# ModelTC/llmc

Hardware: AMD Instinct MI355X
Metric: layers/sec (GPTQ W4A16, Llama-3-8B Linear shapes, 128x2048 calib) (higher is better)
Workload: dtype bf16

## Files before the change

### llmc_amd/_ffi.py

```python
import ctypes as C
import os

import torch

_HERE = os.path.dirname(os.path.abspath(__file__))
LIB_PATH = os.path.join(_HERE, 'csrc', 'libllmc_hip.so')

F16, BF16, F32 = 0, 1, 2
F64 = 3
OUT_FAKE, OUT_I32, OUT_I8, OUT_U8 = 0, 1, 2, 3
SCALAR_QPARAM = 16
LINEAR_YBLOCKED = 4
FRACTIONAL_ZP = 32
KV_REQUANT, KV_NEW_FAKE = 1, 2

_DT = {torch.float16: F16, torch.bfloat16: BF16, torch.float32: F32}

_i64, _i32, _f32, _f64, _vp, _sz = C.c_int64, C.c_int, C.c_float, C.c_double, C.c_void_p, C.c_size_t

SIGNATURES = {
    'llmc_hip_abi_version': (_i32, []),
    'llmc_hip_build_id': (C.c_char_p, []),
    'llmc_hip_last_error': (_i32, [C.c_char_p, _sz]),
    'llmc_hip_set_helper_streams': (_i32, [_i32]),
    'llmc_hip_set_cu_reserve': (_i32, [_i32]),
    'llmc_hip_set_option': (_i32, [C.c_char_p, _i32]),
    'llmc_hip_get_option': (_i32, [C.c_char_p]),
    'llmc_hip_option_name': (_i32, [_i32, C.c_char_p, _sz]),
    'llmc_minmax_qparams_ws_bytes': (_sz, [_i64, _i64]),
    'llmc_minmax_qparams': (_i32, [_vp, _i32, _i64, _i64, _i32, _i32, _f32, _f32, _vp, _vp, _vp, _vp]),
    'llmc_minmax_samples_max': (_i32, []),
    'llmc_minmax_samples_ws_bytes': (_sz, [_vp, _i32]),
    'llmc_minmax_samples': (_i32, [_vp, _vp, _i32, _i32, _vp, _vp, _vp, _vp]),
    'llmc_histc_ws_bytes': (_sz, [_i32]),
    'llmc_histc': (_i32, [_vp, _i32, _i64, _i32, _f32, _f32, _vp, _vp, _vp]),
    'llmc_mse_qparams': (_i32, [_vp, _i32, _i64, _i64, _i32, _i32, _f32, _f32, _i32, _i32, _f32, _vp, _vp, _vp, _vp, _vp]),
    'llmc_mse_qparams_panel': (_i32, [_vp, _i64, _i64, _i64, _i64, _i64, _i32, _i32, _f32, _f32, _i32, _i32, _f32, _vp,
                                      _vp, _i64, _i64, _vp]),
    'llmc_hqq_ws_bytes': (_sz, [_i64, _i64, _i32, _i64, _i32]),
    'llmc_hqq_optimize': (_i32, [_vp, _i32, _i64, _i64, _i64, _i32, _i64, _i32, _i32, _f32, _f32, _vp, _vp, _f32, _f32,
                                 _i32, _i32, _vp, _vp, _vp, _vp, _vp, _vp]),
    'llmc_quant_static': (_i32, [_vp, _i32, _i64, _i64, _vp, _i32, _vp, _i32, _f32, _f32, _i32, _vp, _vp]),
    'llmc_quant_dynamic_ws_bytes': (_sz, [_i64, _i64]),
    'llmc_quant_dynamic': (_i32, [_vp, _i32, _i64, _i64, _i32, _i32, _f32, _f32, _i32, _vp, _vp, _vp, _vp, _vp]),
    'llmc_pack_lsb': (_i32, [_vp, _i32, _i64, _i64, _i32, _vp, _vp]),
    'llmc_hessian_accum_ws_bytes': (_sz, [_i64, _i64, _i64]),
    'llmc_hessian_accum': (_i32, [_vp, _vp, _i32, _i64, _i64, _i64, _f64, _f64, _vp, _vp]),
    'llmc_hessian_accum_partials': (_i32, [_vp, _i32, _i64, _i64, _i64, _vp, _vp]),
    'llmc_hessian_accum_reduce': (_i32, [_vp, _i64, _i64, _i64, _f64, _f64, _vp, _vp]),
    'llmc_hessian_max_samples': (_i32, []),
    'llmc_hessian_accum_ptrs_ws_bytes': (_sz, [_vp, _i32, _i64, _i64]),
    'llmc_hessian_accum_ptrs': (_i32, [_vp, _vp, _vp, _i32, _i32, _i64, _i64, _f64, _f64, _vp, _vp]),
    'llmc_hessian_accum_ptrs_partials': (_i32, [_vp, _vp, _i32, _i32, _i64, _i64, _vp, _vp]),
    'llmc_hessian_accum_ptrs_reduce': (_i32, [_vp, _vp, _i32, _i64, _i64, _f64, _f64, _vp, _vp]),
    'llmc_hessian_accum_barrier_timeouts': (_i32, [_vp, _vp, _i32, _i64, _i64, _vp, _vp]),
    'llmc_hessian_max_problems': (_i32, []),
    'llmc_hessian_accum_multi_ws_bytes': (_sz, [_vp, _i32]),
    'llmc_hessian_accum_multi_partials': (_i32, [_vp, _i32, _i32, _vp, _vp]),
    'llmc_hessian_accum_multi_reduce': (_i32, [_vp, _i32, _vp, _vp]),
    'llmc_hessian_accum_multi_barrier_timeouts': (_i32, [_vp, _i32, _vp, _vp, _vp]),
    'llmc_gather_cols': (_i32, [_vp, _i64, _i64, _vp, _vp, _vp]),
    'llmc_hessian_prep_ws_bytes': (_sz, [_i64]),
    'llmc_hessian_prep': (_i32, [_vp, _vp, _i32, _i64, _i64, _vp, _f32, _vp, _vp, _vp, _vp]),
    'llmc_chol_inv_upper_ws_bytes': (_sz, [_i64]),
    'llmc_chol_inv_upper': (_i32, [_vp, _i64, _vp, _vp, _vp]),
    'llmc_hessian_prep_rev': (_i32, [_vp, _vp, _i32, _i64, _i64, _vp, _f32, _vp, _vp, _vp, _vp]),
    'llmc_chol_inv_upper_rev': (_i32, [_vp, _vp, _i64, _vp, _vp, _vp]),
    'llmc_gptq_quantize_ws_bytes': (_sz, [_i64, _i64]),
    'llmc_gptq_quantize': (_i32, [_vp, _vp, _i64, _i64, _i32, _f32, _f32, _i64, _i32, _vp, _vp, _vp, _vp, _vp,
                                  _i32, _vp, _vp]),
    'llmc_gptq_quantize_cols': (_i32, [_vp, _vp, _i64, _i64, _i64, _i32, _f32, _f32, _i64, _i32, _vp, _vp, _vp, _vp, _vp,
                                       _i32, _vp, _vp]),
    'llmc_gptq_quantize_fp8_cols': (_i32, [_vp, _vp, _i64, _i64, _i64, _i32, _i64, _i32, _vp, _vp, _vp, _vp, _i32, _vp, _vp]),
    'llmc_gptq_quantize_mse_ws_bytes': (_sz, [_i64, _i64]),
    'llmc_gptq_quantize_mse': (_i32, [_vp, _vp, _i64, _i64, _i64, _i32, _f32, _f32, _i64, _i32, _i32, _i32, _f32, _vp, _vp,
                                      _vp, _vp, _i32, _vp, _vp]),
    'llmc_spqr_quantize_ws_bytes': (_sz, [_i64, _i64]),
    'llmc_spqr_quantize': (_i32, [_vp, _vp, _i64, _i64, _f32, _f32, _i64, _f32, _i32, _f32, _f32, _f32, _f32, _vp, _vp,
                                  _vp, _vp, _vp, _i32, _vp, _vp]),
    'llmc_awq_act_mean_ws_bytes': (_sz, [_i64, _i64]),
    'llmc_awq_act_mean': (_i32, [_vp, _i32, _i64, _i64, _vp, _vp, _vp]),
    'llmc_awq_weight_mean_ws_bytes': (_sz, [_i64, _i64]),
    'llmc_awq_weight_mean': (_i32, [_vp, _i32, _i64, _i64, _i64, _vp, _vp, _vp]),
    'llmc_awq_scales': (_i32, [_vp, _vp, _i32, _i64, _f64, _i32, _vp, _vp]),
    'llmc_awq_scale_fakequant': (_i32, [_vp, _vp, _i32, _i64, _i64, _i64, _i32, _f32, _f32, _vp, _vp]),
    'llmc_div_cols': (_i32, [_vp, _vp, _i32, _i64, _i64, _vp, _vp]),
    'llmc_div_cols_kt': (_i32, [_vp, _vp, _i32, _i64, _i64, _vp, _vp]),
    'llmc_mul_cols': (_i32, [_vp, _vp, _i32, _i64, _i64, _vp]),
    'llmc_clamp_groups': (_i32, [_vp, _i32, _i64, _i64, _i64, _vp, _vp, _vp]),
    'llmc_linear_eval_ws_bytes': (_sz, [_i64, _i64, _i64]),
    'llmc_linear_eval': (_i32, [_vp, _vp, _i32, _i64, _i64, _i64, _i32, _vp, _vp, _vp, _vp, _vp]),
    'llmc_linear_eval_yblocked_bytes': (_sz, [_i64, _i64]),
    'llmc_ktile_pack': (_i32, [_vp, _i32, _i64, _i64, _vp, _vp]),
    'llmc_linear_eval_kt': (_i32, [_vp, _vp, _i32, _i64, _i64, _i64, _i32, _vp, _vp, _vp, _vp, _vp]),
    'llmc_awq_clip_search_ws_bytes': (_sz, [_i64, _i64, _i64, _i64]),
    'llmc_awq_clip_search': (_i32, [_vp, _vp, _i32, _i64, _i64, _i64, _i64, _i32, _i32, _i32, _i32, _f32, _f32,
                                    _vp, _vp, _vp, _vp]),
    'llmc_awq_clip_errs': (_i32, [_vp, _vp, _i32, _i64, _i64, _i64, _i64, _i32, _i32, _i32, _i32, _f32, _f32, _vp, _vp]),
    'llmc_awq_clip_errs_cand': (_i32, [_vp, _vp, _vp, _vp, _i32, _i64, _i64, _i64, _i64, _i64, _i32, _vp, _vp]),
    'llmc_fp8_quant_ws_bytes': (_sz, [_i64, _i64]),
    'llmc_fp8_quant': (_i32, [_vp, _i32, _i64, _i64, _i32, _vp, _vp, _i32, _i32, _vp, _vp]),
    'llmc_fpx_quant_ws_bytes': (_sz, [_i64, _i64]),
    'llmc_fpx_quant': (_i32, [_vp, _i32, _i64, _i64, _vp, _i64, _i32, _vp, _vp, _i32, _i32, _vp, _vp]),
    'llmc_fp4_pack': (_i32, [_vp, _i64, _i64, _vp, _vp]),
    'llmc_fpx_dequant': (_i32, [_vp, _i32, _i32, _vp, _i32, _i64, _i64, _vp, _i32, _vp]),
    'llmc_fp8_block_quant': (_i32, [_vp, _i32, _i64, _i64, _i32, _f32, _i32, _vp, _vp, _vp]),
    'llmc_fp8_block_dequant': (_i32, [_vp, _vp, _i64, _i64, _i32, _i32, _vp, _vp]),
    'llmc_fp8_act_quant': (_i32, [_vp, _i32, _i64, _i32, _vp, _vp, _vp]),
    'llmc_fp8_block_gemm': (_i32, [_vp, _vp, _vp, _vp, _i64, _i64, _i64, _i32, _vp, _vp, _vp]),
    'llmc_mx_act_quant': (_i32, [_vp, _i32, _i64, _i64, _i32, _vp, _vp, _vp]),
    'llmc_mx_gemm': (_i32, [_vp, _i32, _vp, _vp, _vp, _i64, _i64, _i64, _i32, _vp, _vp, _vp]),
    'llmc_pack_awq_gemm': (_i32, [_vp, _i32, _vp, _i32, _vp, _i64, _i64, _i64, _vp, _vp, _vp, _vp]),
    'llmc_col_stats_ws_bytes': (_sz, [_i64, _i64]),
    'llmc_col_stats': (_i32, [_vp, _i32, _i64, _i64, _i32, _vp, _vp, _vp, _vp]),
    'llmc_smooth_scales': (_i32, [_vp, _vp, _i32, _i64, _f64, _f64, _vp, _vp]),
    'llmc_osplus_scale': (_i32, [_vp, _vp, _vp, _i64, _i32, _i64, _vp, _vp]),
    'llmc_osplus_act_step_tier': (_i32, [_i32, _i64]),
    'llmc_osplus_act_step': (_i32, [_vp, _vp, _i32, _i64, _i64, _i32, _i32, _f32, _f32, _i32, _vp, _vp]),
    'llmc_quant_dynamic_mixed_fits': (_i32, [_i32, _i64]),
    'llmc_quant_dynamic_mixed': (_i32, [_vp, _i32, _i64, _i64, _vp, _vp, _i64, _i64, _i32, _i32, _f32, _f32, _vp, _vp]),
    'llmc_quant_dynamic_cols_ws_bytes': (_sz, [_i64, _i64, _i64]),
    'llmc_quant_dynamic_cols': (_i32, [_vp, _i32, _i64, _i64, _i64, _i64, _i32, _i32, _f32, _f32, _i32, _vp, _vp, _vp, _vp, _vp]),
    'llmc_quant_dynamic_cols_paths': (_i32, []),
    'llmc_quant_dynamic_cols_path': (_i32, [_vp, _i32, _i64, _i64, _i64, _i64]),
    'llmc_hadamard': (_i32, [_vp, _vp, _i32, _i64, _i64, _i64, _vp, _i32, _f64, _vp]),
    'llmc_col_sqsum_ws_bytes': (_sz, [_i64, _i64, _i32]),
    'llmc_col_sqsum': (_i32, [_vp, _i32, _i64, _i64, _i32, _vp, _vp, _i64, _vp, _vp]),
    'llmc_prune_rows': (_i32, [_vp, _i32, _i64, _i64, _i64, _vp, _i64, _i64, _vp, _vp]),
    'llmc_prune_rows_paths': (_i32, []),
    'llmc_prune_rows_path': (_i32, [_i32, _i64, _i64, _i64, _i64, _vp]),
    'llmc_magnitude_prune_ws_bytes': (_sz, [_i32, _i64, _i64]),
    'llmc_magnitude_prune': (_i32, [_vp, _i32, _i64, _i64, _i64, _i64, _vp, _vp, _vp, _vp]),
    'llmc_sparsegpt_prune_ws_bytes': (_sz, [_i64, _i64]),
    'llmc_sparsegpt_prune': (_i32, [_vp, _vp, _i64, _i64, _f64, _i64, _i64, _vp, _vp, _vp, _i32, _vp, _vp]),
    'llmc_kv_cache_update': (_i32, [_i32, _i64, _i64, _i64, _i64, _i64, _i64, _i64, _i32, _i32, _f32, _f32, _i32, _vp, _vp, _vp,
                                    _vp, _vp, _vp, _vp, _vp, _vp, _vp, _i64, _i64, _i64, _vp]),
    'llmc_kv_sink_update': (_i32, [_i32, _i64, _i64, _i64, _i64, _i64, _i64, _i64, _i64, _i64, _i64, _i64, _vp, _vp, _vp, _vp, _vp,
                                   _vp, _vp, _vp, _i64, _i64, _i64, _vp]),
    'llmc_block_influence_ws_bytes': (_sz, [_i64]),
    'llmc_block_influence': (_i32, [_vp, _vp, _i32, _i64, _i64, _i64, _i64, _i32, _vp, _vp, _vp, _vp]),
    'llmc_cosine_dist_ws_bytes': (_sz, [_i64, _i64]),
    'llmc_cosine_dist': (_i32, [_vp, _i32, _i64, _i64, _i64, _vp, _vp, _vp]),
    'llmc_maxmin_select_max_n': (_i32, []),
    'llmc_maxmin_select_ws_bytes': (_sz, [_i64]),
    'llmc_maxmin_select': (_i32, [_vp, _i32, _i64, _i64, _i64, _vp, _vp, _vp]),
    'llmc_test_sgemm': (_i32, [_vp, _vp, _vp, _i64, _i64, _i64, _i32, _i32, _i32, _i32, _i32, _i32, _i32, _i32,
                               _i32, _i32, _vp]),
    'llmc_test_sgemm_phased': (_i32, [_vp, _vp, _vp, _i64, _i64, _i64, _i32, _i32, _i32, _i32, _i32, _vp]),
    'llmc_test_gemm3': (_i32, [_vp, _vp, _vp, _i64, _i64, _i64, _i32, _i32, _i32, _i32, _i32, _i32, _i32, _i32, _vp]),
    'llmc_test_gemm3_planes': (_i32, [_vp, _vp, _vp, _i64, _i64, _i64, _i32, _i32, _i32, _i32, _i32, _vp, _vp]),
    'llmc_test_gemm3s_stamps': (_i32, [_vp]),
    'llmc_test_gptq_rider_plan': (_i32, [_i64, _i64, _i64, _i64, _i32, _vp, _i32]),
    'llmc_test_gptq_pipe_plan': (_i32, [_i64, _i64, _i64, _i64, _i32, _vp, _i32]),
    'llmc_test_chol_plan': (_i32, [_i64, _i32, _i32, _vp, _i32]),
    'llmc_test_gemm_route': (_i32, [_vp, _vp]),
    'llmc_test_linear_route': (_i32, [_vp, _vp]),
}



class HessianProblem(C.Structure):
    _fields_ = [('H', _vp), ('dstate', _vp), ('X_list_host', _vp), ('T_list_host', _vp), ('n', _i32), ('K', _i64),
                ('ldx', _i64), ('n_before', _f64), ('n_after', _f64)]


_lib = None


class LlmcHipError(RuntimeError):
    pass


def lib():
    global _lib
    if _lib is None:
        if not os.path.exists(LIB_PATH):
            raise LlmcHipError(
                f'{LIB_PATH} not found: the HIP extension is required (run `python -m llmc_amd.build`). '
                'llmc_amd has no CPU fallback.')
        handle = C.CDLL(LIB_PATH)
        for name, (res, args) in SIGNATURES.items():
            fn = getattr(handle, name)
            fn.restype = res
            fn.argtypes = args
        ver = handle.llmc_hip_abi_version()
        if ver != 1:
            raise LlmcHipError(f'libllmc_hip.so ABI version {ver} != 1')
        if not os.environ.get('LLMC_SKIP_BUILD_ID_CHECK'):
            from . import build as _build
            have, want = handle.llmc_hip_build_id().decode(), _build.source_digest()
            if have != want:
                raise LlmcHipError(f'{LIB_PATH} is stale: built from sources {have}, csrc/ is {want} '
                                   '(run `python -m llmc_amd.build`; LLMC_SKIP_BUILD_ID_CHECK=1 skips this check)')
        _lib = handle
        _apply_startup_options()
    return _lib


HOST_OPTIONS = {
    'awq_kt': 1,
    'awq_y_bytes': (1 << 32) - (1 << 20),
    'k3_fused_prep': 1,
    'quant_cols': 1,
}

_HOST_DEFAULTS = dict(HOST_OPTIONS)


def reset_options():
    HOST_OPTIONS.update(_HOST_DEFAULTS)
    if _lib is not None:
        for k in library_options():
            _lib.llmc_hip_set_option(k.encode(), 0)


def set_option(key, value):
    if key in HOST_OPTIONS:
        prev, HOST_OPTIONS[key] = HOST_OPTIONS[key], int(value)
        return prev
    prev = lib().llmc_hip_set_option(key.encode(), int(value))
    if prev < 0:
        raise ValueError(f'unknown option {key!r} (library keys: {library_options()}; host keys: {sorted(HOST_OPTIONS)})')
    return prev


def get_option(key):
    if key in HOST_OPTIONS:
        return HOST_OPTIONS[key]
    v = lib().llmc_hip_get_option(key.encode())
    if v < 0:
        raise ValueError(f'unknown option {key!r}')
    return v


def library_options():
    out, buf, i = [], C.create_string_buffer(64), 0
    while lib().llmc_hip_option_name(i, buf, 64) > 0:
        out.append(buf.value.decode())
        i += 1
    return out


class option:

    def __init__(self, **kv):
        self.kv = kv

    def __enter__(self):
        self.prev = {k: set_option(k, v) for k, v in self.kv.items()}
        return self

    def __exit__(self, *exc):
        for k, v in self.prev.items():
            set_option(k, v)
        return False


def _apply_startup_options():
    spec = os.environ.get('LLMC_OPTIONS', '')
    for item in filter(None, (x.strip() for x in spec.split(','))):
        k, _, v = item.partition('=')
        set_option(k.strip(), int(v or 1))


def last_error():
    buf = C.create_string_buffer(512)
    lib().llmc_hip_last_error(buf, 512)
    return buf.value.decode(errors='replace')


def check(rc, what):
    if rc == 0:
        return
    msg = last_error()
    if rc == -22:
        raise ValueError(f'{what}: invalid argument: {msg}')
    if rc == -95:
        raise NotImplementedError(f'{what}: unsupported: {msg}')
    raise LlmcHipError(f'{what}: HIP error: {msg}')


def dt(t):
    try:
        return _DT[t.dtype if isinstance(t, torch.Tensor) else t]
    except KeyError:
        raise ValueError(f'unsupported dtype {t.dtype if isinstance(t, torch.Tensor) else t}')


def require_gpu(*tensors):
    cur = None
    for t in tensors:
        if t is None:
            continue
        if not t.is_cuda:
            raise LlmcHipError(
                'llmc_amd operators run on MI355X only (tensor is on '
                f'{t.device}); there is no CPU fallback. Use oracle/ for CPU checks in tests.')
        if cur is None:
            cur = torch.cuda.current_device()
        if t.device.index != cur:
            raise LlmcHipError(f'tensor lives on {t.device} but the current device is cuda:{cur}: wrap the call in '
                               '`with torch.cuda.device(tensor.device)` (hipSetDevice is the caller\'s job)')


def ptr(t):
    return 0 if t is None else t.data_ptr()


def stream():
    return torch.cuda.current_stream().cuda_stream


def workspace(nbytes, device):
    if nbytes <= 0:
        return None
    return torch.empty(int(nbytes), dtype=torch.uint8, device=device)


class helper_streams:

    def __init__(self, enable):
        self.enable = int(bool(enable))

    def __enter__(self):
        self.prev = lib().llmc_hip_set_helper_streams(self.enable)

    def __exit__(self, *exc):
        lib().llmc_hip_set_helper_streams(self.prev)
        return False


class cu_reserve:

    def __init__(self, n):
        self.n = int(n)

    def __enter__(self):
        self.prev = lib().llmc_hip_set_cu_reserve(self.n)

    def __exit__(self, *exc):
        lib().llmc_hip_set_cu_reserve(self.prev)
        return False
```

### llmc_amd/csrc/abi.hip

```cpp
#include <mutex>
#include <set>
#include <utility>
#include "common.h"

namespace llmc {
static thread_local char g_last_error[512] = "";
static thread_local int g_helper_streams = 1;
bool helper_streams_enabled() { return g_helper_streams != 0; }
static thread_local int g_cu_reserve = 0;
int cu_reserve() { return g_cu_reserve; }
static thread_local int g_opt[OPT_COUNT] = {};
int opt(int id) { return (id >= 0 && id < OPT_COUNT) ? g_opt[id] : 0; }
static const char* const g_opt_names[OPT_COUNT] = {
    "k3_fp32", "k3_no_gemm6", "k3_no_planes", "k3_split_far", "k4_split_far", "k4_err_rowmajor", "gptq_generic",
    "gemm3_nospec", "gemm3s_min_tiles", "no_shortk", "linear_nosplit", "fp8_exact_div", "side_cu_mask", "k1_batch_off", "k1_fp32_diag", "fp8_no_packed16", "gemm3s_no_dma", "sgemm_no_wide", "gemm3_no_wide", "no_riders", "kv_sink_max_grid",
    "block_influence_max_grid"};

void set_last_error(const char* where, hipError_t e) {
    snprintf(g_last_error, sizeof(g_last_error), "%s: %s (%d)", where, hipGetErrorString(e), (int)e);
}
void set_last_error_msg(const char* msg) { snprintf(g_last_error, sizeof(g_last_error), "%s", msg); }

static std::mutex g_dev_mu;
static int g_cu_count[LLMC_MAX_DEVICES] = {};
static std::set<std::pair<int, const void*>> g_lds_attr_done;

int device_cu_count() {
    int dev = 0;
    if (hipGetDevice(&dev) != hipSuccess || dev < 0 || dev >= LLMC_MAX_DEVICES) return 256;
    std::lock_guard<std::mutex> lk(g_dev_mu);
    if (g_cu_count[dev] == 0) {
        int n = 0;
        if (hipDeviceGetAttribute(&n, hipDeviceAttributeMultiprocessorCount, dev) != hipSuccess || n <= 0) n = 256;
        g_cu_count[dev] = n;
    }
    return g_cu_count[dev];
}

int ensure_dynamic_lds(const void* fn, int bytes) {
    int dev = 0;
    LLMC_HIP_CHECK(hipGetDevice(&dev));
    std::lock_guard<std::mutex> lk(g_dev_mu);
    auto key = std::make_pair(dev, fn);
    if (g_lds_attr_done.count(key)) return LLMC_OK;
    LLMC_HIP_CHECK(hipFuncSetAttribute(fn, hipFuncAttributeMaxDynamicSharedMemorySize, bytes));
    g_lds_attr_done.insert(key);
    return LLMC_OK;
}
}

extern "C" int llmc_hip_set_helper_streams(int enable) {
    int prev = llmc::g_helper_streams;
    llmc::g_helper_streams = enable ? 1 : 0;
    return prev;
}

extern "C" int llmc_hip_set_option(const char* key, int value) {
    if (!key || value < 0) return LLMC_EINVAL;
    for (int i = 0; i < llmc::OPT_COUNT; ++i)
        if (strcmp(key, llmc::g_opt_names[i]) == 0) {
            const int prev = llmc::g_opt[i];
            llmc::g_opt[i] = value;
            return prev;
        }
    llmc::set_last_error_msg("llmc_hip_set_option: unknown key");
    return LLMC_EINVAL;
}

extern "C" int llmc_hip_get_option(const char* key) {
    if (!key) return LLMC_EINVAL;
    for (int i = 0; i < llmc::OPT_COUNT; ++i)
        if (strcmp(key, llmc::g_opt_names[i]) == 0) return llmc::g_opt[i];
    return LLMC_EINVAL;
}

extern "C" int llmc_hip_option_name(int index, char* buf_host, size_t n) {
    if (index < 0 || index >= llmc::OPT_COUNT || !buf_host || n == 0) return LLMC_EINVAL;
    strncpy(buf_host, llmc::g_opt_names[index], n - 1);
    buf_host[n - 1] = 0;
    return (int)strlen(buf_host);
}

extern "C" int llmc_hip_set_cu_reserve(int n_cus) {
    int prev = llmc::g_cu_reserve;
    llmc::g_cu_reserve = n_cus < 0 ? 0 : n_cus;
    return prev;
}

extern "C" int llmc_hip_abi_version(void) { return LLMC_HIP_ABI_VERSION; }

#ifndef LLMC_BUILD_ID
#define LLMC_BUILD_ID "unknown"
#endif
extern "C" const char* llmc_hip_build_id(void) { return LLMC_BUILD_ID; }

extern "C" int llmc_hip_last_error(char* buf_host, size_t n) {
    if (!buf_host || n == 0) return (int)strlen(llmc::g_last_error);
    strncpy(buf_host, llmc::g_last_error, n - 1);
    buf_host[n - 1] = 0;
    return (int)strlen(buf_host);
}
```

### llmc_amd/csrc/cholesky.hip

```cpp
#include <stdlib.h>
#include "common.h"
#include "mfma_common.h"
#include "sgemm.h"
#include "pipe_lanes.h"

namespace llmc {

static constexpr int NB = 128;

__global__ __launch_bounds__(256) void k_antitranspose(const float* __restrict__ in, float* __restrict__ out,
                                                       int n, int upper_only) {
    __shared__ float tile[32][33];
    const int tx = threadIdx.x & 31, ty = threadIdx.x >> 5;
    const int r0 = blockIdx.y * 32, c0 = blockIdx.x * 32;
    for (int y = ty; y < 32; y += 8) {
        int r = r0 + y, c = c0 + tx;
        tile[y][tx] = (r < n && c < n) ? in[(int64_t)r * n + c] : 0.0f;
    }
    __syncthreads();
    for (int y = ty; y < 32; y += 8) {
        int c = c0 + y, r = r0 + tx;
        if (r < n && c < n) {
            int orow = n - 1 - c, ocol = n - 1 - r;
            float v = tile[tx][y];
            if (upper_only && ocol < orow) v = 0.0f;
            out[(int64_t)orow * n + ocol] = v;
        }
    }
}

static constexpr int PLD = 132;

__device__ __forceinline__ float rdlane(float v, int l) {
    return __int_as_float(__builtin_amdgcn_readlane(__float_as_int(v), l));
}

__device__ __forceinline__ void wave_potrf32_inv(float* __restrict__ S, float* __restrict__ V,
                                                 float* __restrict__ rowbuf, int lane, int kglobal,
                                                 int* __restrict__ info) {
#pragma clang fp contract(fast)
    (void)rowbuf;
    const int j = lane & 31, h = lane >> 5;
    f32x16 A, E;
#pragma unroll
    for (int r = 0; r < 16; ++r) {
        const int row = (r & 3) + 8 * (r >> 2) + 4 * h;
        A[r] = S[row * PLD + j];
        E[r] = row == j ? 1.0f : 0.0f;
    }
    bool bad = false;
#pragma unroll
    for (int q = 0; q < 8; ++q) {
        const int rb = 4 * (q >> 1), hq = q & 1;
        const bool mine = h == hq;
        float row[4], va[4], rinv[4], m[4][4];
#pragma unroll
        for (int t = 0; t < 4; ++t) row[t] = A[rb + t];
#pragma unroll
        for (int t = 0; t < 4; ++t) {
            const int i = 4 * q + t;
            const float d = rdlane(row[t], hq * 32 + i);
            if (!(d > 0.0f)) bad = true;
            float ri = __builtin_amdgcn_rsqf(d);
            ri = ri * (1.5f - 0.5f * d * ri * ri);
            rinv[t] = ri;
            va[t] = (mine && j >= i) ? row[t] * ri : 0.0f;
#pragma unroll
            for (int s2 = t + 1; s2 < 4; ++s2) {
                m[t][s2] = rdlane(va[t], hq * 32 + 4 * q + s2);
                row[s2] = __builtin_fmaf(-m[t][s2], va[t], row[s2]);
            }
        }
        float er[4], ve[4];
#pragma unroll
        for (int t = 0; t < 4; ++t) er[t] = E[rb + t];
#pragma unroll
        for (int t = 0; t < 4; ++t) {
            ve[t] = mine ? er[t] * rinv[t] : 0.0f;
#pragma unroll
            for (int s2 = t + 1; s2 < 4; ++s2) er[s2] = __builtin_fmaf(-m[t][s2], ve[t], er[s2]);
        }
#pragma unroll
        for (int t = 0; t < 4; ++t) {
            A[rb + t] = mine ? va[t] : A[rb + t];
            E[rb + t] = mine ? ve[t] : E[rb + t];
        }
        if (q < 7) {
#pragma unroll
            for (int pr = 0; pr < 2; ++pr) {
                const float b0 = va[2 * pr], b1 = va[2 * pr + 1];
                const float e0 = ve[2 * pr], e1 = ve[2 * pr + 1];
                const float a0 = (mine && j >= 4 * q + 4) ? -b0 : 0.0f;
                const float a1 = (mine && j >= 4 * q + 4) ? -b1 : 0.0f;
                float opa, opb, ope;
                if (hq == 0) {
                    opa = __int_as_float(__builtin_amdgcn_permlane32_swap(__float_as_int(a0), __float_as_int(a1), false, false)[0]);
                    opb = __int_as_float(__builtin_amdgcn_permlane32_swap(__float_as_int(b0), __float_as_int(b1), false, false)[0]);
                    ope = __int_as_float(__builtin_amdgcn_permlane32_swap(__float_as_int(e0), __float_as_int(e1), false, false)[0]);
                } else {
                    opa = __int_as_float(__builtin_amdgcn_permlane32_swap(__float_as_int(a1), __float_as_int(a0), false, false)[1]);
                    opb = __int_as_float(__builtin_amdgcn_permlane32_swap(__float_as_int(b1), __float_as_int(b0), false, false)[1]);
                    ope = __int_as_float(__builtin_amdgcn_permlane32_swap(__float_as_int(e1), __float_as_int(e0), false, false)[1]);
                }
                A = __builtin_amdgcn_mfma_f32_32x32x2f32(opa, opb, A, 0, 0, 0);
                E = __builtin_amdgcn_mfma_f32_32x32x2f32(opa, ope, E, 0, 0, 0);
            }
        }
    }
    if (bad && lane == 0) atomicCAS(info, 0, kglobal + 1);
#pragma unroll
    for (int r = 0; r < 16; ++r) {
        const int row = (r & 3) + 8 * (r >> 2) + 4 * h;
        S[row * PLD + j] = j >= row ? A[r] : 0.0f;
    }
#pragma unroll
    for (int q = 0; q < 4; ++q)
        *reinterpret_cast<float4*>(V + j * PLD + 8 * q + 4 * h) = make_float4(E[4 * q], E[4 * q + 1], E[4 * q + 2], E[4 * q + 3]);
}

template <bool TA>
__device__ __forceinline__ f32x16 blk_mm(const float* __restrict__ A, const float* __restrict__ B, f32x16 acc,
                                          int lane) {
    const int c = lane & 31, h = lane >> 5;
#pragma unroll
    for (int kk = 0; kk < 16; ++kk) {
        const int k = 2 * kk + h;
        const float av = TA ? A[k * PLD + c] : A[c * PLD + k];
        const float bv = B[k * PLD + c];
        acc = __builtin_amdgcn_mfma_f32_32x32x2f32(av, bv, acc, 0, 0, 0);
    }
    return acc;
}
__device__ __forceinline__ void blk_store(float* __restrict__ C, const f32x16& acc, int lane, float sign) {
    const int c = lane & 31, h = lane >> 5;
#pragma unroll
    for (int r = 0; r < 16; ++r) C[((r & 3) + 8 * (r >> 2) + 4 * h) * PLD + c] = sign * acc[r];
}
__device__ __forceinline__ void blk_sub(float* __restrict__ C, const f32x16& acc, int lane) {
    const int c = lane & 31, h = lane >> 5;
#pragma unroll
    for (int r = 0; r < 16; ++r) {
        float* p = C + ((r & 3) + 8 * (r >> 2) + 4 * h) * PLD + c;
        *p = *p - acc[r];
    }
}
#define PBLK(M, bi, bj) ((M) + (bi) * 32 * PLD + (bj) * 32)
#define VBLK(a, b) ((a) == (b) ? (Vd + (a) * 32) : PBLK(S, b, a))

#ifdef LLMC_PROBE_STAMPS
__device__ long long g_potrf_stamps[32];
#define LLMC_STAMP(i) do { if (threadIdx.x == 0) g_potrf_stamps[i] = clock64(); } while (0)
#else
#define LLMC_STAMP(i) do { } while (0)
#endif

__global__ __launch_bounds__(256, 2) void k_potrf_inv(float* __restrict__ W, int64_t ld, int k0, int nb,
                                                   float* __restrict__ Vout, int* __restrict__ info) {
    extern __shared__ __attribute__((aligned(16))) float plds[];
    float* S = plds;
    float* Vd = plds + NB * PLD;
    float* rowbuf = plds + NB * PLD + 32 * PLD;
    const int tid = threadIdx.x;
    const int lane = tid & 63;
    const int wv = __builtin_amdgcn_readfirstlane(tid >> 6);
    const f32x16 zero = {0.f, 0.f, 0.f, 0.f, 0.f, 0.f, 0.f, 0.f, 0.f, 0.f, 0.f, 0.f, 0.f, 0.f, 0.f, 0.f};
    LLMC_STAMP(0);
    {
        float4 ld4[16];
        const bool full = nb == NB && (ld % 4 == 0) && (k0 % 4 == 0);
        if (full) {
            const float* base = W + (int64_t)(k0 + (tid >> 5)) * ld + k0 + (tid & 31) * 4;
#pragma unroll
            for (int q = 0; q < 16; ++q) ld4[q] = *reinterpret_cast<const float4*>(base + (int64_t)(8 * q) * ld);
        } else {
#pragma unroll
            for (int q = 0; q < 16; ++q) {
                const int e4 = tid + 256 * q;
                const int i = e4 >> 5, j = (e4 & 31) * 4;
                float4 v = make_float4(0.f, 0.f, 0.f, 0.f);
                if (i < nb) {
                    const float* p = W + (int64_t)(k0 + i) * ld + k0 + j;
                    if (j < nb) v.x = p[0];
                    if (j + 1 < nb) v.y = p[1];
                    if (j + 2 < nb) v.z = p[2];
                    if (j + 3 < nb) v.w = p[3];
                }
                ld4[q] = v;
            }
        }
#pragma unroll
        for (int q = 0; q < 16; ++q) {
            const int e4 = tid + 256 * q;
            const int i = e4 >> 5, j = (e4 & 31) * 4;
            float vv[4] = {ld4[q].x, ld4[q].y, ld4[q].z, ld4[q].w};
#pragma unroll
            for (int t = 0; t < 4; ++t) {
                const int jj = j + t;
                float x = (i == jj) ? 1.0f : 0.0f;
                if (i < nb && jj < nb) x = (jj >= i) ? vv[t] : 0.0f;
                vv[t] = x;
            }
            *reinterpret_cast<float4*>(S + i * PLD + j) = make_float4(vv[0], vv[1], vv[2], vv[3]);
        }
    }
    __syncthreads();
    LLMC_STAMP(1);
    for (int kb = 0; kb < 4; ++kb) {
        if (wv == 0) wave_potrf32_inv(PBLK(S, kb, kb), VBLK(kb, kb), rowbuf, lane, k0 + kb * 32, info);
        __syncthreads();
        LLMC_STAMP(2 + 2 * kb);
        {
            const int jb = kb + 1 + wv;
            if (jb < 4) {
                f32x16 acc = blk_mm<true>(VBLK(kb, kb), PBLK(S, kb, jb), zero, lane);
                blk_store(PBLK(S, kb, jb), acc, lane, 1.0f);
            }
        }
        __syncthreads();
        {
            int idx = 0;
            for (int ib = kb + 1; ib < 4; ++ib)
                for (int jb = ib; jb < 4; ++jb, ++idx)
                    if ((idx & 3) == wv) {
                        f32x16 acc = blk_mm<true>(PBLK(S, kb, ib), PBLK(S, kb, jb), zero, lane);
                        blk_sub(PBLK(S, ib, jb), acc, lane);
                    }
        }
        __syncthreads();
        LLMC_STAMP(3 + 2 * kb);
    }
    if (nb == NB && (ld % 4 == 0) && (k0 % 4 == 0)) {
#pragma unroll
        for (int q = 0; q < 16; ++q) {
            const int e4 = tid + 256 * q;
            const int i = e4 >> 5, j = (e4 & 31) * 4;
            float4 s4 = make_float4(0.f, 0.f, 0.f, 0.f);
            if ((j >> 5) >= (i >> 5)) s4 = *reinterpret_cast<const float4*>(S + i * PLD + j);
            *reinterpret_cast<float4*>(W + (int64_t)(k0 + i) * ld + k0 + j) = s4;
        }
    } else {
        for (int e = tid; e < NB * NB; e += 256) {
            const int i = e >> 7, j = e & 127;
            if (i < nb && j < nb) W[(int64_t)(k0 + i) * ld + k0 + j] = (j >= i) ? S[i * PLD + j] : 0.0f;
        }
    }
    LLMC_STAMP(10);
    if (wv < 2) {
        const int a = 2 * wv, b = a + 1;
        f32x16 x = blk_mm<false>(VBLK(a, a), PBLK(S, a, b), zero, lane);
        blk_store(VBLK(a, b), x, lane, 1.0f);
        f32x16 y = blk_mm<false>(VBLK(a, b), VBLK(b, b), zero, lane);
        blk_store(VBLK(a, b), y, lane, -1.0f);
    }
    __syncthreads();
    {
        const int r = wv >> 1, c = 2 + (wv & 1);
        f32x16 x = blk_mm<false>(VBLK(r, r), PBLK(S, r, c), zero, lane);
        if (r == 0) x = blk_mm<false>(VBLK(0, 1), PBLK(S, 1, c), x, lane);
        __syncthreads();
        blk_store(VBLK(r, c), x, lane, 1.0f);
    }
    __syncthreads();
    {
        const int r = wv >> 1, c = 2 + (wv & 1);
        f32x16 y = blk_mm<false>(VBLK(r, 2), VBLK(2, c), zero, lane);
        if (c == 3) y = blk_mm<false>(VBLK(r, 3), VBLK(3, 3), y, lane);
        blk_store(PBLK(S, r, c), y, lane, -1.0f);
    }
    __syncthreads();
    LLMC_STAMP(11);
#pragma unroll
    for (int q = 0; q < 16; ++q) {
        const int e4 = tid + 256 * q;
        const int i = e4 >> 5, j = (e4 & 31) * 4;
        const int bi = i >> 5, bj = j >> 5;
        float4 v4 = make_float4(0.f, 0.f, 0.f, 0.f);
        if (bi == bj) v4 = *reinterpret_cast<const float4*>(Vd + (i & 31) * PLD + j);
        else if (bi < 2 && bj >= 2) v4 = *reinterpret_cast<const float4*>(S + i * PLD + j);
        else if (bi < bj) v4 = *reinterpret_cast<const float4*>(S + (bj * 32 + (i & 31)) * PLD + bi * 32 + (j & 31));
        *reinterpret_cast<float4*>(Vout + i * NB + j) = v4;
    }
    LLMC_STAMP(12);
}
#undef PBLK

__global__ __launch_bounds__(256) void k_zero_subdiag(float* __restrict__ W, int64_t ld, int K) {
    const int r0 = blockIdx.x * 256 + 128, c0 = blockIdx.x * 256;
    for (int e = threadIdx.x; e < 128 * 128; e += 256) {
        const int i = r0 + (e >> 7), j = c0 + (e & 127);
        if (i < K && j < K) W[(int64_t)i * ld + j] = 0.0f;
    }
}

__global__ __launch_bounds__(256) void k_place_diag_inv(float* __restrict__ W, int64_t ld, int K,
                                                        const float* __restrict__ Vbuf, int b0) {
    const int b = b0 + blockIdx.x;
    const int k0 = b * NB;
    const int nb = min(NB, K - k0);
    const float* V = Vbuf + (int64_t)b * NB * NB;
    for (int e = threadIdx.x; e < NB * NB; e += 256) {
        int i = e >> 7, j = e & 127;
        if (i < nb && j < nb) W[(int64_t)(k0 + i) * ld + k0 + j] = V[e];
    }
}

__global__ __launch_bounds__(1024) void k_diag_fix(float* __restrict__ H, int K, uint8_t* __restrict__ dead,
                                                   float* __restrict__ diag_mean) {
    __shared__ double red[1024];
    double s = 0.0;
    for (int i = threadIdx.x; i < K; i += 1024) {
        float d = H[(int64_t)i * K + i];
        uint8_t dd = (d == 0.0f);
        if (dd) {
            d = 1.0f;
            H[(int64_t)i * K + i] = 1.0f;
        }
        dead[i] = dd;
        s += (double)d;
    }
    red[threadIdx.x] = s;
    __syncthreads();
    for (int o = 512; o > 0; o >>= 1) {
        if (threadIdx.x < o) red[threadIdx.x] += red[threadIdx.x + o];
        __syncthreads();
    }
    if (threadIdx.x == 0) *diag_mean = (float)(red[0] / (double)K);
}

__global__ __launch_bounds__(256) void k_gather_h(const float* __restrict__ H, int K,
                                                  const int64_t* __restrict__ perm, float percdamp,
                                                  const float* __restrict__ diag_mean, float* __restrict__ Hout) {
    const int i = blockIdx.y;
    const int64_t pi = perm ? perm[i] : i;
    const float damp = percdamp * (*diag_mean);
    for (int j = blockIdx.x * 256 + threadIdx.x; j < K; j += gridDim.x * 256) {
        const int64_t pj = perm ? perm[j] : j;
        float v = H[pi * K + pj];
        if (i == j) v += damp;
        Hout[(int64_t)i * K + j] = v;
    }
}

template <typename T>
__global__ __launch_bounds__(256) void k_gather_w(const T* __restrict__ W, int64_t R, int K,
                                                  const int64_t* __restrict__ perm,
                                                  const uint8_t* __restrict__ dead, float* __restrict__ Wout) {
    const int64_t r = blockIdx.y;
    for (int j = blockIdx.x * 256 + threadIdx.x; j < K; j += gridDim.x * 256) {
        const int64_t pj = perm ? perm[j] : j;
        float v = dead[pj] ? 0.0f : to_f32<T>(W[r * K + pj]);
        Wout[r * K + j] = v;
    }
}


template <typename T> __device__ __forceinline__ float4 load4_f32(const T* p);
template <> __device__ __forceinline__ float4 load4_f32<float>(const float* p) {
    return *reinterpret_cast<const float4*>(p);
}
template <> __device__ __forceinline__ float4 load4_f32<f16_t>(const f16_t* p) {
    const uint2 u = *reinterpret_cast<const uint2*>(p);
    f16_t h[4];
    __builtin_memcpy(h, &u, 8);
    return make_float4(to_f32<f16_t>(h[0]), to_f32<f16_t>(h[1]), to_f32<f16_t>(h[2]), to_f32<f16_t>(h[3]));
}
template <> __device__ __forceinline__ float4 load4_f32<bf16_t>(const bf16_t* p) {
    const uint2 u = *reinterpret_cast<const uint2*>(p);
    bf16_t h[4];
    __builtin_memcpy(h, &u, 8);
    return make_float4(to_f32<bf16_t>(h[0]), to_f32<bf16_t>(h[1]), to_f32<bf16_t>(h[2]), to_f32<bf16_t>(h[3]));
}

static constexpr int GATHER_ROWS = 8;
static constexpr int GATHER_MAXJ = 7;
template <typename T, int MODE>
__global__ __launch_bounds__(512) void k_gather_lds(const T* __restrict__ in, int K, const int64_t* __restrict__ idx,
                                                   const uint8_t* __restrict__ dead, float percdamp,
                                                   const float* __restrict__ diag_mean, float* __restrict__ out, int64_t R) {
    extern __shared__ __attribute__((aligned(16))) float grow[];
    const float damp = MODE == 2 ? percdamp * (*diag_mean) : 0.0f;
    const int64_t r_begin = (int64_t)blockIdx.x * GATHER_ROWS;
    const int64_t r_end = r_begin + GATHER_ROWS < R ? r_begin + GATHER_ROWS : R;
    for (int c_pass = 0; c_pass < K; c_pass += 4 * 512 * GATHER_MAXJ) {
        int pj[GATHER_MAXJ][4];
        uint32_t deadbits = 0;
#pragma unroll
        for (int j = 0; j < GATHER_MAXJ; ++j) {
            const int c = c_pass + 4 * (int)threadIdx.x + 4 * 512 * j;
#pragma unroll
            for (int t = 0; t < 4; ++t) {
                int v = 0;
                if (c < K) {
                    v = idx ? (int)idx[c + t] : c + t;
                    if (MODE == 1 && dead[v]) deadbits |= 1u << (4 * j + t);
                }
                pj[j][t] = v;
            }
        }
        for (int64_t r = r_begin; r < r_end; ++r) {
            const int64_t sr = (MODE == 2 && idx) ? idx[r] : r;
            const T* src = in + sr * K;
            __syncthreads();
            for (int c = 4 * threadIdx.x; c < K; c += 4 * 512) *reinterpret_cast<float4*>(grow + c) = load4_f32<T>(src + c);
            __syncthreads();
#pragma unroll
            for (int j = 0; j < GATHER_MAXJ; ++j) {
                const int c = c_pass + 4 * (int)threadIdx.x + 4 * 512 * j;
                if (c >= K) break;
                float v[4];
#pragma unroll
                for (int t = 0; t < 4; ++t) {
                    float x = grow[pj[j][t]];
                    if (MODE == 1 && ((deadbits >> (4 * j + t)) & 1u)) x = 0.0f;
                    if (MODE == 2 && r == c + t) x += damp;
                    v[t] = x;
                }
                *reinterpret_cast<float4*>(out + r * K + c) = make_float4(v[0], v[1], v[2], v[3]);
            }
        }
    }
}

static constexpr int GATHER_LDS_MAX = 160 * 1024;

template <typename T, int MODE>
static int gather_lds_launch(const T* in, int64_t R, int64_t K, const int64_t* idx, const uint8_t* dead,
                             float percdamp, const float* diag_mean, float* out, hipStream_t st) {
    if (K * 4 > 65536)
        if (int rc = ensure_dynamic_lds((const void*)k_gather_lds<T, MODE>, GATHER_LDS_MAX)) return rc;
    hipLaunchKernelGGL((k_gather_lds<T, MODE>), dim3((unsigned)ceil_div64(R, GATHER_ROWS)), dim3(512), (size_t)K * 4, st, in,
                       (int)K, idx, dead, percdamp, diag_mean, out, R);
    LLMC_LAUNCH_CHECK();
    return LLMC_OK;
}
static inline bool gather_lds_ok(int64_t K, const void* in, const void* out, int esz) {
    return K % 4 == 0 && K * 4 <= GATHER_LDS_MAX && ((uintptr_t)in % (4 * esz)) == 0 && ((uintptr_t)out & 15) == 0;
}

}

using namespace llmc;

extern "C" int llmc_gather_cols(const float* in, int64_t R, int64_t K, const int64_t* idx, float* out,
                                llmc_stream_t stream) {
    LLMC_REQUIRE(in && idx && out && R > 0 && K > 0, "gather_cols: null/empty argument");
    LLMC_REQUIRE(in != out, "gather_cols: out must not alias in");
    hipStream_t st = (hipStream_t)stream;
    if (gather_lds_ok(K, in, out, 4))
        return gather_lds_launch<float, 0>(in, R, K, idx, nullptr, 0.0f, nullptr, out, st);
    set_last_error_msg("gather_cols: K must be a multiple of 4 with K <= 40960 and 16-byte aligned rows");
    return LLMC_ENOTSUP;
}

extern "C" size_t llmc_hessian_prep_ws_bytes(int64_t K) {
    if (K <= 0) return 0;
    return (size_t)(((K + 63) / 64) * 64 + 64) + (size_t)K * 8;
}

namespace llmc {
__global__ __launch_bounds__(256) void k_reverse_perm(const int64_t* __restrict__ perm, int K, int64_t* __restrict__ out) {
    const int i = blockIdx.x * 256 + threadIdx.x;
    if (i < K) out[i] = perm ? perm[K - 1 - i] : (int64_t)(K - 1 - i);
}
}

static int hessian_prep_impl(float* H, const void* W, int wdt, int64_t R, int64_t K, const int64_t* perm, float percdamp,
                             float* Hout, float* Wout, void* ws, llmc_stream_t stream, bool rev) {
    LLMC_REQUIRE(H && ws && K > 0, "hessian_prep: null/empty argument");
    LLMC_REQUIRE((W && Wout && R > 0) || (!W && !Wout), "hessian_prep: W and Wout go together");
    LLMC_REQUIRE(dtype_ok(wdt), "hessian_prep: bad dtype");
    LLMC_REQUIRE(Hout != H, "hessian_prep: Hout must not alias H");
    LLMC_REQUIRE(K < (1ll << 31) && R < 65536ll * 32768ll, "hessian_prep: shape too large");
    hipStream_t st = (hipStream_t)stream;
    float* diag_mean = (float*)ws;
    uint8_t* dead = (uint8_t*)ws + 64;
    hipLaunchKernelGGL(k_diag_fix, dim3(1), dim3(1024), 0, st, H, (int)K, dead, diag_mean);
    LLMC_LAUNCH_CHECK();
    int gx = (int)ceil_div64(K, 256 * 4);
    if (Hout) {
        const int64_t* hperm = perm;
        if (rev) {
            int64_t* pr = (int64_t*)((char*)ws + (((K + 63) / 64) * 64 + 64));
            hipLaunchKernelGGL(k_reverse_perm, dim3((unsigned)ceil_div64(K, 256)), dim3(256), 0, st, perm, (int)K, pr);
            LLMC_LAUNCH_CHECK();
            hperm = pr;
        }
        if (gather_lds_ok(K, H, Hout, 4)) {
            int rc = gather_lds_launch<float, 2>(H, K, K, hperm, nullptr, percdamp, diag_mean, Hout, st);
            if (rc) return rc;
        } else {
            hipLaunchKernelGGL(k_gather_h, dim3(gx, (unsigned)K), dim3(256), 0, st, (const float*)H, (int)K, hperm,
                               percdamp, (const float*)diag_mean, Hout);
            LLMC_LAUNCH_CHECK();
        }
    }
    if (W && gather_lds_ok(K, W, Wout, wdt == LLMC_F32 ? 4 : 2)) {
        int rc;
        if (wdt == LLMC_F16) rc = gather_lds_launch<f16_t, 1>((const f16_t*)W, R, K, perm, dead, 0.0f, nullptr, Wout, st);
        else if (wdt == LLMC_BF16)
            rc = gather_lds_launch<bf16_t, 1>((const bf16_t*)W, R, K, perm, dead, 0.0f, nullptr, Wout, st);
        else rc = gather_lds_launch<float, 1>((const float*)W, R, K, perm, dead, 0.0f, nullptr, Wout, st);
        return rc;
    }
    for (int64_t r0 = 0; W && r0 < R; r0 += 32768) {
        int64_t rows = R - r0 < 32768 ? R - r0 : 32768;
        dim3 grid(gx, (unsigned)rows);
        if (wdt == LLMC_F16)
            hipLaunchKernelGGL((k_gather_w<f16_t>), grid, dim3(256), 0, st, (const f16_t*)W + r0 * K, rows, (int)K,
                               perm, (const uint8_t*)dead, Wout + r0 * K);
        else if (wdt == LLMC_BF16)
            hipLaunchKernelGGL((k_gather_w<bf16_t>), grid, dim3(256), 0, st, (const bf16_t*)W + r0 * K, rows, (int)K,
                               perm, (const uint8_t*)dead, Wout + r0 * K);
        else
            hipLaunchKernelGGL((k_gather_w<float>), grid, dim3(256), 0, st, (const float*)W + r0 * K, rows, (int)K,
                               perm, (const uint8_t*)dead, Wout + r0 * K);
        LLMC_LAUNCH_CHECK();
    }
    return LLMC_OK;
}

extern "C" int llmc_hessian_prep(float* H, const void* W, int wdt, int64_t R, int64_t K, const int64_t* perm,
                                 float percdamp, float* Hout, float* Wout, void* ws, llmc_stream_t stream) {
    return hessian_prep_impl(H, W, wdt, R, K, perm, percdamp, Hout, Wout, ws, stream, false);
}

extern "C" int llmc_hessian_prep_rev(float* H, const void* W, int wdt, int64_t R, int64_t K, const int64_t* perm,
                                     float percdamp, float* Hout, float* Wout, void* ws, llmc_stream_t stream) {
    return hessian_prep_impl(H, W, wdt, R, K, perm, percdamp, Hout, Wout, ws, stream, true);
}

static inline size_t align256(size_t x) { return (x + 255) & ~(size_t)255; }

static constexpr int64_t GEMM6_MIN_H = 4096;
static size_t gemm6_bytes(int64_t K) {
    size_t mx = 0;
    for (int64_t h = NB; h < K; h *= 2)
        if (h >= GEMM6_MIN_H) {
            const size_t b = gemm6_ws_bytes((int)h, (int)h, (int)h);
            if (b > mx) mx = b;
        }
    return align256(mx);
}

struct FactorWs { size_t work, vbuf, xbuf, xbuf_bytes, g6, total; };
static FactorWs factor_ws(int64_t K) {
    FactorWs w{};
    w.vbuf = align256((size_t)K * K * 4);
    w.xbuf = w.vbuf + align256((size_t)ceil_div64(K, NB) * NB * NB * 4);
    w.xbuf_bytes = (size_t)(K / 2 + NB) * (K / 2 + NB) * 4;
    w.g6 = w.xbuf + align256(w.xbuf_bytes);
    w.total = w.g6 + gemm6_bytes(K);
    return w;
}

extern "C" size_t llmc_chol_inv_upper_ws_bytes(int64_t K) { return K <= 0 ? 0 : factor_ws(K).total; }

static constexpr int NBO = 4 * NB;
struct Piece { int a0, a1; Lane lane; };
static int step_pieces(int c1, int oend, int K, bool piped, Piece* p) {
    if (!piped || oend >= K) return p[0] = Piece{c1, K, CHAIN}, 1;
    return p[0] = Piece{c1, oend, CHAIN}, p[1] = Piece{oend, K, BULK}, 2;
}
static int far_pieces(int oend, int K, bool merged, Piece* p) {
    if (merged || oend + NBO >= K) return p[0] = Piece{oend, K, CHAIN}, 1;
    return p[0] = Piece{oend, oend + NBO, CHAIN}, p[1] = Piece{oend + NBO, K, BULK}, 2;
}

struct Level { int64_t h, stride, ldX; int npairs, n2_last; bool x3, g6; };
struct FactorCall {
    float* Wk; float* Vbuf; float* Xbuf; void* G6buf; int K; size_t xbuf_bytes;
    bool x3, planes, merge_far, g6;
    float* at(int64_t r, int64_t c) const { return Wk + r * K + c; }
    float* V(int c0) const { return Vbuf + (size_t)(c0 / NB) * NB * NB; }
    static SgemmArgs one(int M, int N, int Kd, int epilogue) {
        SgemmArgs g{};
        g.M = g.M_last = M; g.N = g.N_last = N; g.Kd = g.Kd_last = Kd; g.epilogue = epilogue; g.batch = 1;
        return g;
    }
    SgemmArgs panel_solve(int c0, int nb, int col0, int col1) const {
        SgemmArgs g = one(nb, col1 - col0, nb, SG_SET);
        g.A = V(c0); g.lda = NB; g.B = g.C = at(c0, col0); g.ldb = g.ldc = K; g.a_lower = 1;
        return g;
    }
    SgemmArgs inblock_update(int c0, int nb, int oend, int col0, int col1) const {
        SgemmArgs u = one(oend - (c0 + nb), col1 - col0, nb, SG_SUB);
        u.A = at(c0, c0 + nb); u.B = at(c0, col0); u.C = at(c0 + nb, col0); u.lda = u.ldb = u.ldc = K;
        u.c_upper_only = col0 == c0 + nb ? 1 : 0;
        return u;
    }
    SgemmArgs far(int k0, int oend, int r0, int r1, bool with_planes) const {
        SgemmArgs u = one(r1 - r0, K - r0, oend - k0, SG_SUB);
        u.A = u.B = at(k0, r0); u.C = at(r0, r0); u.lda = u.ldb = u.ldc = K; u.c_upper_only = 1;
        if (with_planes) {
            u.planesA = u.planesB = (const uint16_t*)Xbuf + (r0 - oend);
            u.ldp = K - oend; u.plane_stride = (int64_t)(oend - k0) * (K - oend);
        }
        return u;
    }
    bool split_planes(int k0, int oend, int r0) const {
        const int nfar = K - oend;
        return x3 && planes && nfar % 8 == 0 && (size_t)3 * (oend - k0) * nfar * 2 <= xbuf_bytes && gemm3_route(far(k0, oend, r0, K, true), true).planes();
    }
    Level level(int64_t h) const {
        Level l{h, 2 * h * ((int64_t)K + 1), h, (int)((K - h + 2 * h - 1) / (2 * h)), 0, false, false};
        if (l.npairs <= 0) return l;
        const int64_t rest = K - (int64_t)(l.npairs - 1) * 2 * h - h;
        l.n2_last = (int)(rest < h ? rest : h);
        if (l.npairs == 1) l.ldX = ((l.n2_last + 3) / 4) * 4;
        l.x3 = x3 && h >= 512;
        l.g6 = l.x3 && g6 && h >= GEMM6_MIN_H && h % 256 == 0 && l.n2_last % 256 == 0;
        return l;
    }
    SgemmArgs level_x(const Level& l) const {
        SgemmArgs x = one((int)l.h, (int)l.h, (int)l.h, SG_SET);
        x.A = Wk; x.B = Wk + l.h; x.lda = x.ldb = K; x.sA = x.sB = l.stride; x.C = Xbuf; x.ldc = l.ldX; x.sC = l.h * l.h;
        x.N_last = l.n2_last; x.a_upper = 1; x.batch = l.npairs;
        return x;
    }
    SgemmArgs level_c(const Level& l) const {
        SgemmArgs y = one((int)l.h, (int)l.h, (int)l.h, SG_NEG);
        y.A = Xbuf; y.lda = l.ldX; y.sA = l.h * l.h; y.B = Wk + l.h * ((int64_t)K + 1); y.C = Wk + l.h; y.ldb = y.ldc = K; y.sB = y.sC = l.stride;
        y.N_last = y.Kd_last = l.n2_last; y.b_upper = 1; y.batch = l.npairs;
        return y;
    }
    static SgemmArgs problem(SgemmArgs g, int z) {
        g.A += z * g.sA; g.B += z * g.sB; g.C += z * g.sC;
        if (z == g.batch - 1) g.M = g.M_last, g.N = g.N_last, g.Kd = g.Kd_last;
        g.batch = 1;
        return g;
    }
};

enum { CP_TRANSPOSE = 0, CP_POTRF = 1, CP_SOLVE = 2, CP_UPDATE = 3, CP_SPLIT = 4, CP_FAR = 7, CP_PLACE = 8, CP_ZERO = 9, CP_INV_X = 10,
       CP_INV_C = 11, CP_W = 22 };
enum { F_KERNEL = 0, F_SGEMM = 1, F_GEMM3 = 2, F_GEMM6 = 3 };
struct Rect { int32_t buf, r0, r1, c0, c1; };
static const int32_t CP_BLANK[CP_W] = {0, 0, -1, 0, 0, 0, 0, -1, 0, 0, 0, 0, -1, 0, 0, 0, 0, -1, 0, 0, 0, 0};
static constexpr int POTRF_LDS = (NB * PLD + 32 * PLD + 64) * (int)sizeof(float);
static int launched() { LLMC_LAUNCH_CHECK(); return LLMC_OK; }
struct FactorSink {
    const FactorCall& o; const Lanes& ln; PlanRec* rec; const float* other; const char* ws_end; int32_t* info;
    Rect rect(const void* p, int64_t ld, int64_t rows, int64_t cols) const {
        const float* f = (const float*)p;
        if ((const char*)f >= (const char*)o.Xbuf && (const char*)f < ws_end) {
            const bool x = (const void*)f < o.G6buf;
            const int64_t off = f - (x ? o.Xbuf : (const float*)o.G6buf);
            return Rect{x ? 2 : 3, 0, 1, (int32_t)off, (int32_t)(off + (rows - 1) * ld + cols)};
        }
        const bool v = f >= o.Vbuf && f < o.Xbuf, w = f >= o.Wk && f < o.Wk + (size_t)o.K * o.K;
        const int64_t n = v ? NB : o.K, off = f - (v ? o.Vbuf : w ? o.Wk : other);
        return Rect{ld != n ? -2 : v ? 1 : w ? 0 : 4, (int32_t)(off / n), (int32_t)(off / n + rows), (int32_t)(off % n), (int32_t)(off % n + cols)};
    }
    int add(int kind, int form, Lane lane, Rect w, Rect a = Rect{-1}, Rect b = Rect{-1}, Rect w2 = Rect{-1}) const {
        int32_t v[CP_W] = {kind, form};
        memcpy(v + 2, &w, sizeof w), memcpy(v + 7, &a, sizeof a), memcpy(v + 12, &b, sizeof b), memcpy(v + 17, &w2, sizeof w2);
        rec->row(v, ln.lane_of(ln.s[lane]));
        return LLMC_OK;
    }
    int transpose(const float* in, float* out, int upper_only) const {
        if (rec) return add(CP_TRANSPOSE, F_KERNEL, CHAIN, rect(out, o.K, o.K, o.K), rect(in, o.K, o.K, o.K));
        hipLaunchKernelGGL(k_antitranspose, dim3((o.K + 31) / 32, (o.K + 31) / 32), dim3(256), 0, ln.s[CHAIN], in, out, o.K, upper_only);
        return launched();
    }
    int potrf(int c0, int nb) const {
        float* Vb = o.V(c0);
        if (rec) return add(CP_POTRF, F_KERNEL, CHAIN, rect(o.at(c0, c0), o.K, nb, nb), rect(o.at(c0, c0), o.K, nb, nb), Rect{-1}, rect(Vb, NB, nb, NB));
        hipLaunchKernelGGL(k_potrf_inv, dim3(1), dim3(256), POTRF_LDS, ln.s[CHAIN], o.Wk, (int64_t)o.K, c0, nb, Vb, info);
        return launched();
    }
    int product(int kind, const SgemmArgs& g, int form, bool TA, Lane lane) const {
        if (g.M <= 0 || g.N <= 0) return LLMC_OK;
        const hipStream_t st = ln.s[lane];
        if (!rec) return form == F_SGEMM ? sgemm_launch(g, TA, false, st) : gemm3_launch(g, TA, st);
        auto hull = [&](const float* p, int64_t ld, int64_t s, int r, int c, int rl, int cl) {
            const Rect a = rect(p, ld, r, c), b = rect(p + (g.batch - 1) * s, ld, rl, cl);
            return Rect{a.buf, a.r0, b.r1, a.c0, b.c1};
        };
        auto planes = [&](const void* p, int n) { return rect(p, 1, 1, (2 * g.plane_stride + (g.Kd - 1) * g.ldp + n + 1) / 2); };
        const bool pl = form == F_GEMM3 && gemm3_route(g, TA).planes();
        return add(kind, form, lane, hull(g.C, g.ldc, g.sC, g.M, g.N, g.M_last, g.N_last),
                   pl ? planes(g.planesA, g.M) : TA ? hull(g.A, g.lda, g.sA, g.Kd, g.M, g.Kd_last, g.M_last) : hull(g.A, g.lda, g.sA, g.M, g.Kd, g.M_last, g.Kd_last),
                   pl ? planes(g.planesB, g.N) : hull(g.B, g.ldb, g.sB, g.Kd, g.N, g.Kd_last, g.N_last));
    }
    int split(int k0, int oend) const {
        const int nbo = oend - k0, nfar = o.K - oend;
        if (rec) return add(CP_SPLIT, F_KERNEL, CHAIN, rect(o.Xbuf, 1, 1, ((int64_t)3 * nbo * nfar + 1) / 2), rect(o.at(k0, oend), o.K, nbo, nfar));
        return gemm3_split_planes(o.at(k0, oend), o.K, nbo, nfar, o.Xbuf, nfar, (int64_t)nbo * nfar, ln.s[CHAIN]);
    }
    int gemm6(int kind, const SgemmArgs& g) const {
        if (rec) return add(kind, F_GEMM6, CHAIN, rect(g.C, g.ldc, g.M, g.N), rect(g.A, g.lda, g.M, g.Kd), rect(g.B, g.ldb, g.Kd, g.N),
                            rect(o.G6buf, 1, 1, (int64_t)(gemm6_ws_bytes(g.M, g.N, g.Kd) / 4)));
        return gemm6_launch(g.A, g.lda, g.B, g.ldb, g.C, g.ldc, g.M, g.N, g.Kd, g.a_upper, g.b_upper, g.epilogue == SG_NEG ? -1.0f : 1.0f,
                            o.G6buf, ln.s[CHAIN]);
    }
    int place_diag() const {
        const int nblk = (o.K + NB - 1) / NB;
        if (rec) return add(CP_PLACE, F_KERNEL, CHAIN, rect(o.Wk, o.K, o.K, o.K), rect(o.Vbuf, NB, (int64_t)nblk * NB, NB));
        hipLaunchKernelGGL(k_place_diag_inv, dim3(nblk), dim3(256), 0, ln.s[CHAIN], o.Wk, (int64_t)o.K, o.K, (const float*)o.Vbuf, 0);
        return launched();
    }
    int zero_subdiag() const {
        if (rec) return add(CP_ZERO, F_KERNEL, CHAIN, rect(o.Wk, o.K, o.K, o.K));
        hipLaunchKernelGGL(k_zero_subdiag, dim3((o.K + 255) / 256), dim3(256), 0, ln.s[CHAIN], o.Wk, (int64_t)o.K, o.K);
        return launched();
    }
};

static int chol_inv_upper_impl(float* A, float* Uout, int64_t K64, void* ws, int32_t* info_dev, llmc_stream_t stream, PlanRec* rec = nullptr) {
    LLMC_REQUIRE(A && ws && info_dev && K64 > 0, "chol_inv_upper: null/empty argument");
    LLMC_REQUIRE(K64 % 4 == 0 && K64 < (1 << 30), "chol_inv_upper: K must be a multiple of 4");
    LLMC_REQUIRE(((uintptr_t)A & 15) == 0 && ((uintptr_t)ws & 255) == 0, "chol_inv_upper: alignment");
    const int K = (int)K64;
    const bool rev = Uout != nullptr;
    const FactorWs l = factor_ws(K);
    char* const w = (char*)ws;
    const FactorCall o{rev ? A : (float*)(w + l.work), (float*)(w + l.vbuf), (float*)(w + l.xbuf), w + l.g6, K, l.xbuf_bytes,
                       !opt(OPT_K3_FP32), !opt(OPT_K3_NO_PLANES), !opt(OPT_K3_SPLIT_FAR), !opt(OPT_K3_NO_GEMM6)};
    Lanes ln((hipStream_t)stream, rec);
    const FactorSink sink{o, ln, rec, rev ? Uout : A, w + l.total, info_dev};
    LLMC_TRY(ln.fork());
    if (!rec) {
        LLMC_HIP_CHECK(hipMemsetAsync(info_dev, 0, 4, ln.s[CHAIN]));
        LLMC_TRY(ensure_dynamic_lds((const void*)k_potrf_inv, POTRF_LDS));
    }
    if (!rev) LLMC_TRY(sink.transpose(A, o.Wk, 0));
    Piece pc[2];
    Ev planes_read{};
    for (int k0 = 0; k0 < K; k0 += NBO) {
        const int oend = k0 + NBO < K ? k0 + NBO : K;
        for (int c0 = k0; c0 < oend; c0 += NB) {
            const int nb = K - c0 < NB ? K - c0 : NB;
            LLMC_TRY(sink.potrf(c0, nb));
            if (c0 + nb >= K) break;
            const int np = step_pieces(c0 + nb, oend, K, ln.piped(), pc);
            LLMC_TRY(sink.product(CP_SOLVE, o.panel_solve(c0, nb, pc[0].a0, pc[0].a1), F_SGEMM, true, CHAIN));
            if (np > 1) {
                LLMC_TRY(ln.order(CHAIN, BULK));
                LLMC_TRY(sink.product(CP_SOLVE, o.panel_solve(c0, nb, pc[1].a0, pc[1].a1), F_SGEMM, true, BULK));
                LLMC_TRY(sink.product(CP_UPDATE, o.inblock_update(c0, nb, oend, pc[1].a0, pc[1].a1), F_SGEMM, true, BULK));
            }
            LLMC_TRY(sink.product(CP_UPDATE, o.inblock_update(c0, nb, oend, pc[0].a0, pc[0].a1), F_SGEMM, true, CHAIN));
        }
        if (oend >= K) break;
        LLMC_TRY(ln.order(BULK, CHAIN));
        const int np = far_pieces(oend, K, !ln.piped() && o.x3 && o.merge_far, pc);
        const bool planes = o.split_planes(k0, oend, pc[np - 1].a0);
        if (planes) {
            LLMC_TRY(ln.wait(CHAIN, planes_read));
            LLMC_TRY(sink.split(k0, oend));
        }
        for (int i = 0; i < np; ++i) {
            if (pc[i].lane == BULK) LLMC_TRY(ln.order(CHAIN, BULK));
            LLMC_TRY(sink.product(CP_FAR, o.far(k0, oend, pc[i].a0, pc[i].a1, planes), o.x3 ? F_GEMM3 : F_SGEMM, true, pc[i].lane));
            if (pc[i].lane == BULK) LLMC_TRY(ln.record(BULK, &planes_read));
        }
    }
    LLMC_TRY(sink.place_diag());
    if (o.x3 && o.g6 && K > GEMM6_MIN_H) LLMC_TRY(sink.zero_subdiag());
    for (int64_t h = NB; h < K; h *= 2) {
        const Level lv = o.level(h);
        if (lv.npairs <= 0) break;
        for (int z = 0; lv.g6 && z < lv.npairs; ++z) {
            LLMC_TRY(sink.gemm6(CP_INV_X, o.problem(o.level_x(lv), z)));
            LLMC_TRY(sink.gemm6(CP_INV_C, o.problem(o.level_c(lv), z)));
        }
        if (lv.g6) continue;
        LLMC_TRY(sink.product(CP_INV_X, o.level_x(lv), lv.x3 ? F_GEMM3 : F_SGEMM, false, CHAIN));
        LLMC_TRY(sink.product(CP_INV_C, o.level_c(lv), lv.x3 ? F_GEMM3 : F_SGEMM, false, CHAIN));
    }
    LLMC_TRY(sink.transpose(o.Wk, rev ? Uout : A, 1));
    return ln.join();
}

extern "C" int llmc_chol_inv_upper(float* A, int64_t K64, void* ws, int32_t* info_dev, llmc_stream_t stream) {
    return chol_inv_upper_impl(A, nullptr, K64, ws, info_dev, stream);
}

extern "C" int llmc_chol_inv_upper_rev(float* Arev, float* Uout, int64_t K64, void* ws, int32_t* info_dev, llmc_stream_t stream) {
    LLMC_REQUIRE(Uout && Uout != Arev && ((uintptr_t)Uout & 15) == 0, "chol_inv_upper_rev: Uout must be a separate 16-B aligned buffer");
    return chol_inv_upper_impl(Arev, Uout, K64, ws, info_dev, stream);
}

extern "C" int llmc_test_chol_plan(int64_t K, int rev, int with_lanes, int32_t* out, int cap) {
    LLMC_REQUIRE(out && cap >= 0, "chol plan: null output");
    PlanRec rec{out, cap, 0, CP_W, with_lanes != 0, CP_BLANK};
    float* const base = (float*)(uintptr_t)((uint64_t)1 << 40);
    const size_t span = (size_t)1 << 36;
    const int rc = chol_inv_upper_impl(base, rev ? base + span : nullptr, K, base + 2 * span, (int32_t*)(base + 3 * span), nullptr, &rec);
    return rc ? rc : rec.n;
}
```

### llmc_amd/csrc/common.h

```cpp
#pragma once
#include <hip/hip_runtime.h>
#include <stdint.h>
#include <string.h>
#include <stdio.h>
#include <stdlib.h>
#include <type_traits>

#include "../../include/llmc_hip.h"

namespace llmc {

void set_last_error(const char* where, hipError_t e);
void set_last_error_msg(const char* msg);

#define LLMC_HIP_CHECK(expr)                                   \
    do {                                                       \
        hipError_t _e = (expr);                                \
        if (_e != hipSuccess) {                                \
            ::llmc::set_last_error(#expr, _e);                 \
            return LLMC_EIO;                                   \
        }                                                      \
    } while (0)

#define LLMC_LAUNCH_CHECK()                                    \
    do {                                                       \
        hipError_t _e = hipGetLastError();                     \
        if (_e != hipSuccess) {                                \
            ::llmc::set_last_error("kernel launch", _e);       \
            return LLMC_EIO;                                   \
        }                                                      \
    } while (0)

#define LLMC_REQUIRE(cond, msg)                                \
    do {                                                       \
        if (!(cond)) {                                         \
            ::llmc::set_last_error_msg(msg);                   \
            return LLMC_EINVAL;                                \
        }                                                      \
    } while (0)

static constexpr int LLMC_MAX_DEVICES = 64;
int device_cu_count();
int ensure_dynamic_lds(const void* fn, int bytes);
int cu_reserve();
bool helper_streams_enabled();

enum Opt : int {
    OPT_K3_FP32 = 0,
    OPT_K3_NO_GEMM6,
    OPT_K3_NO_PLANES,
    OPT_K3_SPLIT_FAR,
    OPT_K4_SPLIT_FAR,
    OPT_K4_ERR_ROWMAJOR,
    OPT_GPTQ_GENERIC,
    OPT_GEMM3_NOSPEC,
    OPT_GEMM3S_MIN_TILES,
    OPT_NO_SHORTK,
    OPT_LINEAR_NOSPLIT,
    OPT_FP8_EXACT_DIV,
    OPT_SIDE_CU_MASK,
    OPT_K1_BATCH_OFF,
    OPT_K1_FP32_DIAG,
    OPT_FP8_NO_PACKED16,
    OPT_GEMM3S_NO_DMA,
    OPT_SGEMM_NO_WIDE,
    OPT_GEMM3_NO_WIDE,
    OPT_NO_RIDERS,
    OPT_KV_SINK_MAX_GRID,
    OPT_BLOCK_INFLUENCE_MAX_GRID,
    OPT_COUNT
};
int opt(int id);
#ifdef LLMC_LAB
static inline const char* lab_env(const char* k) { return getenv(k); }
#endif

static inline int dtype_size(int dt) { return dt == LLMC_F32 ? 4 : 2; }
static inline bool dtype_ok(int dt) { return dt == LLMC_F16 || dt == LLMC_BF16 || dt == LLMC_F32; }

struct f16_t { uint16_t u; };
struct bf16_t { uint16_t u; };

template <typename T> struct dt_of;
template <> struct dt_of<f16_t> { static constexpr int value = LLMC_F16; };
template <> struct dt_of<bf16_t> { static constexpr int value = LLMC_BF16; };
template <> struct dt_of<float> { static constexpr int value = LLMC_F32; };

#define DISPATCH_DT(dt, ...)                                              \
    switch (dt) {                                                         \
        case LLMC_F16: { using T = ::llmc::f16_t; __VA_ARGS__; break; }   \
        case LLMC_BF16: { using T = ::llmc::bf16_t; __VA_ARGS__; break; } \
        default: { using T = float; __VA_ARGS__; break; }                 \
    }
#define DISPATCH_OUT_KIND(kind, ...)                                                     \
    switch (kind) {                                                                      \
        case LLMC_OUT_FAKE: { constexpr int KIND = LLMC_OUT_FAKE; __VA_ARGS__; break; }  \
        case LLMC_OUT_I32: { constexpr int KIND = LLMC_OUT_I32; __VA_ARGS__; break; }    \
        case LLMC_OUT_I8: { constexpr int KIND = LLMC_OUT_I8; __VA_ARGS__; break; }      \
        case LLMC_OUT_U8: { constexpr int KIND = LLMC_OUT_U8; __VA_ARGS__; break; }      \
    }

__device__ __forceinline__ float f16_bits_to_f32(uint16_t u) {
    _Float16 h;
    __builtin_memcpy(&h, &u, 2);
    return (float)h;
}
__device__ __forceinline__ uint16_t f32_to_f16_bits(float v) {
    asm volatile("" : "+v"(v));
    _Float16 h = (_Float16)v;
    uint16_t u;
    __builtin_memcpy(&u, &h, 2);
    return u;
}
__device__ __forceinline__ float bf16_bits_to_f32(uint16_t u) {
    return __uint_as_float(((uint32_t)u) << 16);
}
__device__ __forceinline__ uint16_t f32_to_bf16_bits(float v) {
    const __bf16 h = (__bf16)v;
    uint16_t u;
    __builtin_memcpy(&u, &h, 2);
    return u;
}

__device__ __forceinline__ float opaque_f32(float v) {
    asm volatile("" : "+v"(v));
    return v;
}

__device__ __forceinline__ float rnd(float v, int dt) {
    if (dt == LLMC_F16) return f16_bits_to_f32(f32_to_f16_bits(v));
    if (dt == LLMC_BF16) return bf16_bits_to_f32(f32_to_bf16_bits(v));
    return v;
}
template <int DT> __device__ __forceinline__ float rndc(float v) {
    if constexpr (DT == LLMC_F16) return f16_bits_to_f32(f32_to_f16_bits(v));
    else if constexpr (DT == LLMC_BF16) return bf16_bits_to_f32(f32_to_bf16_bits(v));
    else return v;
}

__device__ __forceinline__ float load_as_f32(const void* p, int64_t i, int dt) {
    if (dt == LLMC_F16) return f16_bits_to_f32(((const uint16_t*)p)[i]);
    if (dt == LLMC_BF16) return bf16_bits_to_f32(((const uint16_t*)p)[i]);
    return ((const float*)p)[i];
}
__device__ __forceinline__ void store_from_f32(void* p, int64_t i, int dt, float v) {
    if (dt == LLMC_F16) ((uint16_t*)p)[i] = f32_to_f16_bits(v);
    else if (dt == LLMC_BF16) ((uint16_t*)p)[i] = f32_to_bf16_bits(v);
    else ((float*)p)[i] = v;
}

template <typename T> __device__ __forceinline__ float to_f32(T v);
template <> __device__ __forceinline__ float to_f32<f16_t>(f16_t v) { return f16_bits_to_f32(v.u); }
template <> __device__ __forceinline__ float to_f32<bf16_t>(bf16_t v) { return bf16_bits_to_f32(v.u); }
template <> __device__ __forceinline__ float to_f32<float>(float v) { return v; }

template <typename T> __device__ __forceinline__ T from_f32(float v);
template <> __device__ __forceinline__ f16_t from_f32<f16_t>(float v) { return f16_t{f32_to_f16_bits(v)}; }
template <> __device__ __forceinline__ bf16_t from_f32<bf16_t>(float v) { return bf16_t{f32_to_bf16_bits(v)}; }
template <> __device__ __forceinline__ float from_f32<float>(float v) { return v; }

__host__ __device__ __forceinline__ int promote(int a, int b) {
    if (a == b) return a;
    return LLMC_F32;
}

__device__ __forceinline__ float wave_max(float v, int width) {
    for (int o = width >> 1; o > 0; o >>= 1) v = fmaxf(v, __shfl_xor(v, o, 64));
    return v;
}
__device__ __forceinline__ float wave_min(float v, int width) {
    for (int o = width >> 1; o > 0; o >>= 1) v = fminf(v, __shfl_xor(v, o, 64));
    return v;
}
__device__ __forceinline__ float wave_sum(float v, int width) {
    for (int o = width >> 1; o > 0; o >>= 1) v += __shfl_xor(v, o, 64);
    return v;
}

template <int I, int N, typename F> __device__ __forceinline__ void static_for(F&& f) {
    if constexpr (I < N) {
        f(std::integral_constant<int, I>{});
        static_for<I + 1, N>(f);
    }
}

static inline int64_t ceil_div64(int64_t a, int64_t b) { return (a + b - 1) / b; }
static inline int capped_grid(int64_t items, int64_t per_block, int64_t cap) {
    const int64_t b = ceil_div64(items, per_block);
    return (int)(b < 1 ? 1 : (b > cap ? cap : b));
}
static inline int pow2_ceil(int64_t x) {
    int p = 1;
    while (p < x) p <<= 1;
    return p;
}

}
```

### llmc_amd/csrc/gemm3_wide.hip

```cpp
#include "mfma_common.h"
#include "sgemm.h"

namespace llmc {
namespace {

constexpr int G_ROW = G_B * 2;
constexpr int G_PLANE = G_K * G_ROW;
constexpr int G_OPND = 3 * G_PLANE;
constexpr int G_SLOT = 2 * G_OPND;
constexpr int G_SLOTS = 3;
static_assert(G_LDS == G_SLOTS * G_SLOT, "72 KiB");
constexpr int G_PER_XCD = 64;

struct G3wArgs {
    const uint16_t* PA;
    const uint16_t* PB;
    float* C;
    int64_t ldc;
    uint32_t row2, ps2, rowC;
    uint32_t bytesP, bytesC;
    int nst;
    int tm, tn, sbm, nsb, sm_log, sn_log;
    int upper;
};

__global__ __launch_bounds__(256, 2) void k_gemm3w(const G3wArgs a) {
    extern __shared__ __attribute__((aligned(16))) char smem_g[];
    const int w = blockIdx.x;
    const int g = (w / (8 * G_PER_XCD)) * 8 + (w & 7);
    if (g >= a.nsb) return;
    const int within = (w >> 3) % G_PER_XCD;
    const int ti = ((g % a.sbm) << a.sm_log) + (within >> a.sn_log), tj = ((g / a.sbm) << a.sn_log) + (within & ((1 << a.sn_log) - 1));
    if (ti >= a.tm || tj >= a.tn) return;
    if (a.upper && tj < ti) return;

    const int tid = threadIdx.x, lane = tid & 63;
    const int wv = __builtin_amdgcn_readfirstlane(tid >> 6);
    const int wm = wv >> 1, wn = wv & 1;
#if defined(G3W_DBG) && G3W_DBG == 1
    const auto dA = uniform_rsrc(a.PA, a.bytesP);
    const auto dB = uniform_rsrc(a.PB, a.bytesP);
#else
    const auto dA = uniform_rsrc(a.PA + (int64_t)ti * G_B, a.bytesP);
    const auto dB = uniform_rsrc(a.PB + (int64_t)tj * G_B, a.bytesP);
#endif
    const auto dC = uniform_rsrc(a.C + (int64_t)ti * G_B * a.ldc + (int64_t)tj * G_B, a.bytesC);
    LDS_AS char* lds = (LDS_AS char*)smem_g;
    const uint32_t lds0 = (uint32_t)(uintptr_t)lds;
    const int nst = a.nst;

    uint32_t vo;
    {
        const int r = lane >> 4, c = lane & 15;
        const int cs = (((c >> 2) ^ r) << 2) | (c & 3);
        vo = (uint32_t)r * a.row2 + (uint32_t)cs * 16u;
    }
    auto issue = [&](int j, uint32_t slot_off) {
        const uint32_t k0 = (uint32_t)j * G_K;
#pragma unroll
        for (int t = 0; t < 6; ++t) {
            const int op = t / 3, pl = t % 3;
            const uint32_t so = (uint32_t)pl * a.ps2 + (k0 + 4u * (uint32_t)wv) * a.row2;
            const uint32_t dst = lds0 + slot_off + (uint32_t)op * G_OPND + (uint32_t)pl * G_PLANE + (uint32_t)wv * 1024u;
            if (op == 0) dma16_to(dA, vo, so, dst); else dma16_to(dB, vo, so, dst);
        }
    };

    const int p = lane & 15;
    const int trow = 8 * (lane >> 5) + (p >> 2);
    const int sub = 32 * ((lane >> 4) & 1) + 8 * (p & 3);
    int offA[2], offB[2];
#pragma unroll
    for (int b = 0; b < 2; ++b) {
        offA[b] = trow * G_ROW + (((2 * wm + b) ^ (p >> 2)) << 6) + sub;
        offB[b] = G_OPND + trow * G_ROW + (((2 * wn + b) ^ (p >> 2)) << 6) + sub;
    }
    s16x8 fa[2][2][3], fb[2][2][3];
    auto rd = [&](auto setc, auto fc, LDS_AS char* base) {
        constexpr int S = decltype(setc)::value, f = decltype(fc)::value;
        constexpr int grp = f >> 2, e = f & 3, b = e & 1;
        constexpr bool isA = grp == 0 ? e >= 2 : e < 2;
        constexpr int pl = grp == 0 ? (isA ? 2 : 0) : grp == 1 ? (isA ? 0 : 2) : 1;
        if constexpr (isA) fa[S][b][pl] = tr_frag<G_ROW>(base + offA[b], pl * G_PLANE);
        else fb[S][b][pl] = tr_frag<G_ROW>(base + offB[b], pl * G_PLANE);
    };

    f32x16 acc[2][2];
#pragma unroll
    for (int m = 0; m < 2; ++m)
#pragma unroll
        for (int n = 0; n < 2; ++n)
#pragma unroll
            for (int r = 0; r < 16; ++r) acc[m][n][r] = 0.0f;

    issue(0, 0);
    issue(1, G_SLOT);
    issue(2, 2 * G_SLOT);
    vm_wait<12>();
    __builtin_amdgcn_s_barrier();
    static_for<0, 12>([&](auto fc) { rd(std::integral_constant<int, 0>{}, fc, lds); });
    __builtin_amdgcn_sched_barrier(0);

    const uint32_t voC = (uint32_t)(wm * 64 + 4 * (lane >> 5)) * a.rowC + (uint32_t)(wn * 64 + (lane & 31)) * 4u;
    auto soC = [&](uint32_t rowC, int m, int n, int r) { return (uint32_t)(m * 32 + (r & 3) + 8 * (r >> 2)) * rowC + (uint32_t)n * 128u; };
    f32x16 oldc[2][2];
    uint32_t cur = 0;
    auto stage = [&](auto setc, auto cbc, auto youngc, int j) {
        constexpr int S = decltype(setc)::value, CB = decltype(cbc)::value, YOUNG = decltype(youngc)::value;
        if (j + 2 < nst) vm_wait<YOUNG>(); else vm_wait<0>();
        __builtin_amdgcn_s_barrier();
#if !(defined(G3W_DBG) && G3W_DBG == 2)
        if (j + 3 < nst) issue(j + 3, cur);
#endif
        const uint32_t nxt = cur + G_SLOT == G_LDS ? 0u : cur + G_SLOT;
        LDS_AS char* nb = lds + nxt;
        __builtin_amdgcn_sched_barrier(0);
        static_for<0, 24>([&](auto ic) {
            constexpr int i = decltype(ic)::value, q = i >> 2, m = (i >> 1) & 1, n = i & 1;
            constexpr int TA = q == 0 ? 2 : q == 1 ? 0 : q == 2 ? 1 : q == 3 ? 1 : 0;
            constexpr int TB = q == 0 ? 0 : q == 1 ? 2 : q == 2 ? 1 : q == 3 ? 0 : q == 4 ? 1 : 0;
            acc[m][n] = Mfma<LLMC_BF16>::run(fa[S][m][TA], fb[S][n][TB], acc[m][n]);
            if constexpr (i < 12) rd(std::integral_constant<int, S ^ 1>{}, std::integral_constant<int, i>{}, nb);
#if !(defined(G3W_DBG) && G3W_DBG == 3)
            if constexpr (CB >= 0 && i >= 12 && i < 20) {
#pragma unroll
                for (int e = 0; e < 2; ++e) {
                    constexpr int r0 = 2 * (i - 12);
                    oldc[CB >> 1][CB & 1][r0 + e] = __builtin_bit_cast(float, __builtin_amdgcn_raw_buffer_load_b32(dC, voC, soC(a.rowC, CB >> 1, CB & 1, r0 + e), 0));
                }
            }
#endif
            __builtin_amdgcn_sched_barrier(0);
        });
        cur = nxt;
    };
    constexpr std::integral_constant<int, 0> S0{};
    constexpr std::integral_constant<int, 1> S1{};
    constexpr std::integral_constant<int, -1> NOC{};
    stage(S0, std::integral_constant<int, 0>{}, std::integral_constant<int, 6>{}, 0);
    stage(S1, std::integral_constant<int, 1>{}, std::integral_constant<int, 22>{}, 1);
    stage(S0, std::integral_constant<int, 2>{}, std::integral_constant<int, 38>{}, 2);
    stage(S1, std::integral_constant<int, 3>{}, std::integral_constant<int, 38>{}, 3);
    stage(S0, NOC, std::integral_constant<int, 38>{}, 4);
    stage(S1, NOC, std::integral_constant<int, 22>{}, 5);
    for (int j = 6; j < nst; j += 2) {
        stage(S0, NOC, std::integral_constant<int, 6>{}, j);
        stage(S1, NOC, std::integral_constant<int, 6>{}, j + 1);
    }

    uint32_t rowC2 = a.rowC;
    asm volatile("" : "+s"(rowC2));
#pragma unroll
    for (int m = 0; m < 2; ++m)
#pragma unroll
        for (int n = 0; n < 2; ++n) {
            if (a.upper && ti == tj && 2 * wn + n < 2 * wm + m) continue;
#if defined(G3W_DBG) && G3W_DBG == 3
            if (acc[m][n][0] != 12345.678f) continue;
#endif
#pragma unroll
            for (int r = 0; r < 16; ++r) {
                const float v = oldc[m][n][r] - acc[m][n][r];
                __builtin_amdgcn_raw_buffer_store_b32(__builtin_bit_cast(unsigned, v), dC, voC, soC(rowC2, m, n, r), 0);
            }
        }
}

}

int gemm3w_launch(const SgemmArgs& a, const GemmRoute& r, hipStream_t st) {
    G3wArgs w{};
    w.PA = (const uint16_t*)a.planesA; w.PB = (const uint16_t*)a.planesB; w.C = a.C; w.ldc = a.ldc;
    w.row2 = (uint32_t)(a.ldp * 2); w.ps2 = (uint32_t)(a.plane_stride * 2); w.rowC = (uint32_t)(a.ldc * 4);
    w.bytesP = (uint32_t)((2 * a.plane_stride + (int64_t)(a.Kd - 1) * a.ldp + G_B) * 2);
    w.bytesC = (uint32_t)(((int64_t)(G_B - 1) * a.ldc + G_B) * 4);
    w.nst = a.Kd / G_K;
    w.tm = a.M / G_B; w.tn = a.N / G_B;
    w.upper = a.c_upper_only ? 1 : 0;
    w.sm_log = r.sm_log; w.sn_log = r.sn_log; w.sbm = r.sbm; w.nsb = r.nsb;
    if (int rc = ensure_dynamic_lds((const void*)k_gemm3w, G_LDS)) return rc;
    hipLaunchKernelGGL(k_gemm3w, dim3(r.gx), dim3(r.threads), G_LDS, st, w);
    LLMC_LAUNCH_CHECK();
    return LLMC_OK;
}

}
```

### llmc_amd/csrc/gemm_route.hip

```cpp
#include "sgemm_wide_tile.h"

namespace llmc {
namespace {
GemmRoute refuse(GemmRoute r, int status, const char* msg) { r.status = status; r.msg = msg; return r; }
GemmRoute tiles(GemmRoute r, int kernel, const SgemmArgs& a, int bm, int bn, bool one_row = false) {
    r.kernel = kernel; r.gx = (a.N + bn - 1) / bn; r.gy = one_row ? 1 : (a.M + bm - 1) / bm; r.gz = a.batch;
    return r;
}
GemmRoute tile_blocks(GemmRoute r, int kernel, int tm, int tn, int logt, bool upper, int lds) {
    int best_cost = 1 << 30;
    for (int sm = 1; sm < logt; ++sm) {
        const int SM = 1 << sm, SN = 1 << (logt - sm);
        const int sbm = (tm + SM - 1) / SM, sbn = (tn + SN - 1) / SN;
        int load[8] = {0, 0, 0, 0, 0, 0, 0, 0};
        for (int g = 0; g < sbm * sbn; ++g) {
            const int i0 = (g % sbm) * SM, j0 = (g / sbm) * SN;
            for (int i = i0; i < i0 + SM && i < tm; ++i) {
                const int jlo = upper && i > j0 ? i : j0, jhi = j0 + SN < tn ? j0 + SN : tn;
                if (jhi > jlo) load[g & 7] += jhi - jlo;
            }
        }
        int mx = 0;
        for (int x = 0; x < 8; ++x) mx = load[x] > mx ? load[x] : mx;
        const int cost = mx * 64 + (SM + SN);
        if (cost < best_cost) { best_cost = cost; r.sm_log = sm; }
    }
    r.sn_log = logt - r.sm_log;
    r.sbm = (tm + (1 << r.sm_log) - 1) >> r.sm_log;
    r.nsb = r.sbm * ((tn + (1 << r.sn_log) - 1) >> r.sn_log);
    r.kernel = kernel; r.lds = lds; r.gx = (unsigned)((r.nsb + 7) / 8 * 8) << logt; r.gy = r.gz = 1;
    return r;
}
int wide_form(const SgemmArgs& a, bool TA, bool TB) {
    if (!TA || TB || a.batch != 1 || a.epilogue != SG_SUB || a.phase_len != 128) return 0;
    if (a.a_upper || a.a_lower || a.b_upper || a.c_upper_only) return 0;
    if (a.M % 128 || a.N % wide::W_BN || a.Kd % 128 || a.Kd < 128 || ((uintptr_t)a.C & 3)) return 0;
    const int64_t lim = (int64_t)1 << 31;
    if ((int64_t)a.Kd * a.lda * 4 >= lim || (int64_t)a.Kd * a.ldb * 4 >= lim || (int64_t)256 * a.ldc * 4 >= lim) return 0;
    if ((const void*)a.C == (const void*)a.A || (const void*)a.C == (const void*)a.B) return 0;
    const int v = opt(OPT_SGEMM_NO_WIDE);
    return v == 1 ? 0 : v == 4 && a.M % 256 == 0 ? 4 : 2;
}
bool gemm3s_eligible(const SgemmArgs& a) {
    if (opt(OPT_GEMM3_NOSPEC)) return false;
    if (a.a_upper || a.a_lower || a.b_upper) return false;
    if ((((uintptr_t)a.C) & 15) || a.ldc % 4 || a.sC % 4) return false;
    if ((int64_t)S_BM * a.ldc * 4 >= (int64_t)0x7fffff00) return false;
    const int64_t kd = a.Kd > a.Kd_last ? a.Kd : a.Kd_last;
    const bool pre = a.planesA != nullptr;
    if (a.Kd % (2 * G3K) || a.Kd_last % (2 * G3K) || a.Kd < 4 * G3K || a.Kd_last < 4 * G3K) return false;
    if (pre && (a.batch != 1 || a.ldp % 8 || a.plane_stride % 8 || (((uintptr_t)a.planesA | (uintptr_t)a.planesB) & 15))) return false;
    const int64_t extent = pre ? (2 * a.plane_stride + (kd + G3K) * a.ldp) * 2 : (kd + G3K) * (a.lda > a.ldb ? a.lda : a.ldb) * 4;
    if (extent >= (int64_t)0x7fffff00) return false;
    const int64_t tm = (a.M + S_BM - 1) / S_BM, tn = (a.N + S_BN - 1) / S_BN;
    const int64_t tiles = a.c_upper_only ? tm * tn - tm * (tm - 1) : tm * tn;
    const int mt = opt(OPT_GEMM3S_MIN_TILES);
    const int min_tiles = mt > 0 ? mt : (pre ? 48 : 256);
    return tiles * a.batch >= min_tiles;
}
bool gemm3w_eligible(const SgemmArgs& a) {
    if (opt(OPT_GEMM3_NO_WIDE)) return false;
    if (!a.planesA || !a.planesB || a.epilogue != SG_SUB || a.M % G_B || a.N % G_B) return false;
    if ((2 * a.plane_stride + ((int64_t)a.Kd + G_K) * a.ldp) * 2 >= (int64_t)0x7fffff00 || (int64_t)G_B * a.ldc * 4 >= (int64_t)0x7fffff00) return false;
    const int64_t tm = a.M / G_B, tn = a.N / G_B;
    const int64_t tiles = a.c_upper_only ? tm * tn - tm * (tm - 1) / 2 : tm * tn;
    const int mt = opt(OPT_GEMM3S_MIN_TILES);
    return tiles >= (mt > 0 ? mt : 1024);
}

}
GemmRoute sgemm_route(const SgemmArgs& a, bool TA, bool TB) {
    GemmRoute r{}; r.threads = 256; r.ta = TA; r.tb = TB; r.phase_len = a.phase_len;
    if (a.M <= 0 || a.N <= 0 || a.batch <= 0) { r.empty = true; return r; }
    if ((a.lda % 4) || (a.ldb % 4) || ((uintptr_t)a.A & 15) || ((uintptr_t)a.B & 15) || (a.sA % 4) || (a.sB % 4))
        return refuse(r, LLMC_EINVAL, "sgemm: operands must be 16-B aligned with ld % 4 == 0");
    r.wide_form = wide_form(a, TA, TB);
    const bool in_place = (const void*)a.C == (const void*)a.B;
    const bool shortk = !TB && a.batch == 1 && !a.a_upper && !a.b_upper && !opt(OPT_NO_SHORTK);
    if (shortk && a.Kd <= SKD && (a.phase_len == 0 || a.phase_len >= a.Kd)) return tiles(r, GK_SHORTK, a, SB, SB, in_place);
    r.phased = true;
    if (shortk && a.epilogue == SG_SUB && a.phase_len == SKD && a.Kd % SKD == 0 && a.Kd > SKD && !a.a_lower &&
        (int64_t)((a.M + SB - 1) / SB) * ((a.N + SB - 1) / SB) <= 1024)
        return tiles(r, GK_SHORTK_PHASED, a, SB, SB);
    if (r.wide_form == 4) return tile_blocks(r, GK_WIDE4, a.M / 256, a.N / wide::W_BN, 5, false, wide::Wide<4>::LDS);
    if (r.wide_form == 2) return tile_blocks(r, GK_WIDE2, a.M / 128, a.N / wide::W_BN, 6, false, wide::Wide<2>::LDS);
    if (in_place && (a.M > GB || a.batch != 1)) return refuse(r, LLMC_EINVAL, "sgemm: in-place C = op(A) B needs a single row tile (M <= 128)");
    if (a.phase_len == 0 && a.epilogue == SG_SUB && !a.a_upper && !TB) r.phase_len = 1 << 30;
    r.phased = r.phase_len > 0;
    if (r.phased && (r.phase_len % GK || a.epilogue != SG_SUB || a.a_upper)) return refuse(r, LLMC_EINVAL, "sgemm: bad phased configuration");
    if (r.phased && TB) return refuse(r, LLMC_ENOTSUP, "sgemm: phased mode supports op(B) = N only");
    auto whole = [&](int M, int N, int Kd) { return M % GB == 0 && N % GB == 0 && Kd % GK == 0; };
    r.edge = !(whole(a.M, a.N, a.Kd) && whole(a.M_last, a.N_last, a.Kd_last));
    return tiles(r, GK_SGEMM, a, GB, GB);
}

GemmRoute gemm3_route(const SgemmArgs& a, bool TA) {
    GemmRoute r{}; r.threads = 256; r.ta = TA;
    if (a.M <= 0 || a.N <= 0 || a.batch <= 0) { r.empty = true; return r; }
    if (a.phase_len != 0) return refuse(r, LLMC_EINVAL, "gemm3: no phased mode");
    if ((a.lda % 4) || (a.ldb % 4) || (a.N % 4) || (a.N_last % 4) || (TA && (a.M % 4 || a.M_last % 4)) || ((uintptr_t)a.A & 15) ||
        ((uintptr_t)a.B & 15) || (a.sA % 4) || (a.sB % 4))
        return refuse(r, LLMC_EINVAL, "gemm3: operands must be 16-B aligned with ld and sizes multiples of 4");
    if ((const void*)a.C == (const void*)a.B || (const void*)a.C == (const void*)a.A) return refuse(r, LLMC_EINVAL, "gemm3: no in-place product");
    if (!TA || !gemm3s_eligible(a)) return tiles(r, GK_GEMM3, a, G3B, G3B);
    if (gemm3w_eligible(a)) return tile_blocks(r, GK_GEMM3W, a.M / G_B, a.N / G_B, 6, a.c_upper_only != 0, G_LDS);
    r.threads = 512; r.lds = S_LDS; r.planes_dma = opt(OPT_GEMM3S_NO_DMA) ? 0 : 1;
    return tiles(r, a.planesA ? GK_GEMM3S_PRE : GK_GEMM3S, a, S_BM, S_BN);
}

}

extern "C" int llmc_test_gemm_route(const int64_t* in, int32_t* out) {
    if (!in || !out) return LLMC_EINVAL;
    char* const base = (char*)(uintptr_t)((uint64_t)1 << 40);
    const size_t span = (size_t)1 << 36;
    llmc::SgemmArgs a{};
    a.M = (int)in[1]; a.N = (int)in[2]; a.Kd = (int)in[3]; a.lda = in[4]; a.ldb = in[5]; a.ldc = in[6];
    a.epilogue = (int)in[9]; a.a_upper = (int)in[10]; a.a_lower = (int)in[11]; a.b_upper = (int)in[12]; a.c_upper_only = (int)in[13];
    a.phase_len = (int)in[14]; a.batch = (int)in[15]; a.M_last = (int)in[16]; a.N_last = (int)in[17]; a.Kd_last = (int)in[18];
    a.sA = in[19]; a.sB = in[20]; a.sC = in[21]; a.ldp = in[23]; a.plane_stride = in[24];
    a.A = (const float*)(base + in[26]); a.B = (const float*)(base + span + in[27]);
    a.C = in[25] == 1 ? (float*)a.B : in[25] == 2 ? (float*)a.A : (float*)(base + 2 * span + in[28]);
    if (in[22]) a.planesA = base + 3 * span + in[29], a.planesB = base + 4 * span + in[29];
    const llmc::GemmRoute r = in[0] ? llmc::gemm3_route(a, in[7] != 0) : llmc::sgemm_route(a, in[7] != 0, in[8] != 0);
    const int32_t v[18] = {r.status, r.kernel, (int32_t)r.gx, (int32_t)r.gy, (int32_t)r.gz, r.threads, r.lds, r.ta, r.tb, r.phased, r.edge,
                           r.phase_len, r.planes_dma, r.sm_log, r.sn_log, r.sbm, r.nsb, r.wide_form};
    memcpy(out, v, sizeof v);
    return r.empty ? 1 : 0;
}
```

### llmc_amd/csrc/sgemm.h

```cpp
#pragma once
#include "common.h"

namespace llmc {

enum SgemmEpilogue { SG_SUB = 0 , SG_SET = 1 , SG_NEG = 2  };

struct SgemmArgs {
    const float* A;
    const float* B;
    float* C;
    int64_t lda, ldb, ldc;
    int M, N, Kd;
    int epilogue;
    int a_upper;
    int a_lower;
    int b_upper;
    int c_upper_only;
    int phase_len;
    int64_t sA, sB, sC;
    int batch;
    int M_last, N_last, Kd_last;
    const void* planesA;
    const void* planesB;
    int64_t ldp, plane_stride;
    int planes_dma;
};

enum GemmKernel { GK_SGEMM, GK_SHORTK, GK_SHORTK_PHASED, GK_WIDE2, GK_WIDE4, GK_GEMM3, GK_GEMM3S, GK_GEMM3S_PRE, GK_GEMM3W };
constexpr int GB = 128, GK = 16, SB = 64, SKD = 128;
constexpr int G3B = 128, G3K = 32, S_BM = 256, S_BN = 128, S_LDS = 144 * 1024;
constexpr int G_B = 128, G_K = 16, G_LDS = 72 * 1024;
struct GemmRoute {
    int status; const char* msg;
    int kernel;
    bool empty;
    unsigned gx, gy, gz; int threads, lds;
    bool ta, tb, phased, edge;
    int phase_len;
    int planes_dma;
    int sm_log, sn_log, sbm, nsb;
    int wide_form;
    bool planes() const { return status == LLMC_OK && !empty && (kernel == GK_GEMM3S_PRE || kernel == GK_GEMM3W); }
};
GemmRoute sgemm_route(const SgemmArgs& a, bool TA, bool TB);
GemmRoute gemm3_route(const SgemmArgs& a, bool TA);
int sgemm_launch(const SgemmArgs& a, bool TA, bool TB, hipStream_t st);
int gemm3_launch(const SgemmArgs& a, bool TA, hipStream_t st);
int sgemm_wide_launch(const SgemmArgs& a, const GemmRoute& r, hipStream_t st);
int gemm3w_launch(const SgemmArgs& a, const GemmRoute& r, hipStream_t st);
int gemm3_split_planes(const float* P, int64_t ld, int rows, int n, void* planes, int64_t ldp, int64_t plane_stride, hipStream_t st);

size_t gemm6_ws_bytes(int M, int N, int Kd);
int gemm6_launch(const float* A, int64_t lda, const float* B, int64_t ldb, float* C, int64_t ldc, int M, int N, int Kd,
                 int a_upper, int b_upper, float sign, void* ws, hipStream_t st);

}
```

Before: 78.80.

## Run far-update GEMM tiles as riders alongside the blocked Cholesky panel factor

Adds a k_potrf_inv_riders kernel in which block 0 runs the single-block panel factor/inverse and the other blocks execute queued gemm3w tiles of the trailing far update. The tail rows of the far update are cut off and dealt out across the following potrf launches. The goal is to fill the idle CUs during the serial one-block potrf steps. It adds a rider queue and planner, an option k3_no_riders, and a plan-recording format. The cost is extra launch-argument size and scheduling complexity.

```diff
diff --git a/llmc_amd/_ffi.py b/llmc_amd/_ffi.py
--- a/llmc_amd/_ffi.py
+++ b/llmc_amd/_ffi.py
@@ -153,6 +153,7 @@
     'llmc_test_gptq_rider_plan': (_i32, [_i64, _i64, _i64, _i64, _i32, _vp, _i32]),
     'llmc_test_gptq_pipe_plan': (_i32, [_i64, _i64, _i64, _i64, _i32, _vp, _i32]),
     'llmc_test_chol_plan': (_i32, [_i64, _i32, _i32, _vp, _i32]),
+    'llmc_test_chol_rider_plan': (_i32, [_i64, _i32, _i32, _vp, _i32]),
     'llmc_test_gemm_route': (_i32, [_vp, _vp]),
     'llmc_test_linear_route': (_i32, [_vp, _vp]),
 }
diff --git a/llmc_amd/csrc/abi.hip b/llmc_amd/csrc/abi.hip
--- a/llmc_amd/csrc/abi.hip
+++ b/llmc_amd/csrc/abi.hip
@@ -13,7 +13,7 @@
 int opt(int id) { return (id >= 0 && id < OPT_COUNT) ? g_opt[id] : 0; }
 static const char* const g_opt_names[OPT_COUNT] = {
     "k3_fp32", "k3_no_gemm6", "k3_no_planes", "k3_split_far", "k4_split_far", "k4_err_rowmajor", "gptq_generic",
-    "gemm3_nospec", "gemm3s_min_tiles", "no_shortk", "linear_nosplit", "fp8_exact_div", "side_cu_mask", "k1_batch_off", "k1_fp32_diag", "fp8_no_packed16", "gemm3s_no_dma", "sgemm_no_wide", "gemm3_no_wide", "no_riders", "kv_sink_max_grid",
+    "gemm3_nospec", "gemm3s_min_tiles", "no_shortk", "linear_nosplit", "fp8_exact_div", "side_cu_mask", "k1_batch_off", "k1_fp32_diag", "fp8_no_packed16", "gemm3s_no_dma", "sgemm_no_wide", "gemm3_no_wide", "no_riders", "k3_no_riders", "kv_sink_max_grid",
     "block_influence_max_grid"};
 
 void set_last_error(const char* where, hipError_t e) {
diff --git a/llmc_amd/csrc/chol_riders_plan.h b/llmc_amd/csrc/chol_riders_plan.h
--- /dev/null
+++ b/llmc_amd/csrc/chol_riders_plan.h
@@ -0,0 +1,37 @@
+#pragma once
+#include <stdint.h>
+
+namespace llmc {
+
+constexpr int RIDERS_CAP = 320;
+constexpr int RIDER_CARRIERS = 4;
+constexpr int RIDER_TILE = 128, RIDER_BLOCK = RIDER_CARRIERS * RIDER_TILE;
+constexpr int RIDER_QUEUE_MAX = RIDER_CARRIERS * RIDERS_CAP;
+
+static inline int rider_rows(int K, int oend, int per_launch, int min_share) {
+    const int per = per_launch < RIDERS_CAP ? per_launch : RIDERS_CAP;
+    const int room = (K - oend - RIDER_BLOCK) / RIDER_TILE;
+    if (per <= 0 || room <= 0) return 0;
+    int T = 0;
+    while (T < 255 && T < room && (T + 1) * (T + 2) / 2 <= RIDER_CARRIERS * per) ++T;
+    return T * (T + 1) / 2 < RIDER_CARRIERS * min_share ? 0 : T;
+}
+
+static inline int rider_queue(int T, uint16_t* q) {
+    int n = 0;
+    for (int bi = 0; bi < T; bi += 4)
+        for (int bj = bi / 8 * 8; bj < T; bj += 8)
+            for (int i = bi; i < bi + 4 && i < T; ++i)
+                for (int j = bj > i ? bj : i; j < bj + 8 && j < T; ++j) q[n++] = (uint16_t)(i << 8 | j);
+    return n;
+}
+
+static inline int rider_share(int left, int carriers) { return carriers <= 0 ? 0 : (left + carriers - 1) / carriers; }
+
+static inline void rider_deal(const uint16_t* q, int n, uint16_t* tile) {
+    int i = 0;
+    for (int x = 0; x < 8; ++x)
+        for (int s = x ? x : 8; s <= n; s += 8) tile[s - 1] = q[i++];
+}
+
+}
diff --git a/llmc_amd/csrc/cholesky.hip b/llmc_amd/csrc/cholesky.hip
--- a/llmc_amd/csrc/cholesky.hip
+++ b/llmc_amd/csrc/cholesky.hip
@@ -2,6 +2,8 @@
 #include "common.h"
 #include "mfma_common.h"
 #include "sgemm.h"
+#include "gemm3w_tile.h"
+#include "chol_riders_plan.h"
 #include "pipe_lanes.h"
 
 namespace llmc {
@@ -157,130 +159,27 @@
 __global__ __launch_bounds__(256, 2) void k_potrf_inv(float* __restrict__ W, int64_t ld, int k0, int nb,
                                                    float* __restrict__ Vout, int* __restrict__ info) {
     extern __shared__ __attribute__((aligned(16))) float plds[];
-    float* S = plds;
-    float* Vd = plds + NB * PLD;
-    float* rowbuf = plds + NB * PLD + 32 * PLD;
-    const int tid = threadIdx.x;
-    const int lane = tid & 63;
-    const int wv = __builtin_amdgcn_readfirstlane(tid >> 6);
-    const f32x16 zero = {0.f, 0.f, 0.f, 0.f, 0.f, 0.f, 0.f, 0.f, 0.f, 0.f, 0.f, 0.f, 0.f, 0.f, 0.f, 0.f};
-    LLMC_STAMP(0);
-    {
-        float4 ld4[16];
-        const bool full = nb == NB && (ld % 4 == 0) && (k0 % 4 == 0);
-        if (full) {
-            const float* base = W + (int64_t)(k0 + (tid >> 5)) * ld + k0 + (tid & 31) * 4;
-#pragma unroll
-            for (int q = 0; q < 16; ++q) ld4[q] = *reinterpret_cast<const float4*>(base + (int64_t)(8 * q) * ld);
-        } else {
-#pragma unroll
-            for (int q = 0; q < 16; ++q) {
-                const int e4 = tid + 256 * q;
-                const int i = e4 >> 5, j = (e4 & 31) * 4;
-                float4 v = make_float4(0.f, 0.f, 0.f, 0.f);
-                if (i < nb) {
-                    const float* p = W + (int64_t)(k0 + i) * ld + k0 + j;
-                    if (j < nb) v.x = p[0];
-                    if (j + 1 < nb) v.y = p[1];
-                    if (j + 2 < nb) v.z = p[2];
-                    if (j + 3 < nb) v.w = p[3];
-                }
-                ld4[q] = v;
-            }
-        }
-#pragma unroll
-        for (int q = 0; q < 16; ++q) {
-            const int e4 = tid + 256 * q;
-            const int i = e4 >> 5, j = (e4 & 31) * 4;
-            float vv[4] = {ld4[q].x, ld4[q].y, ld4[q].z, ld4[q].w};
-#pragma unroll
-            for (int t = 0; t < 4; ++t) {
-                const int jj = j + t;
-                float x = (i == jj) ? 1.0f : 0.0f;
-                if (i < nb && jj < nb) x = (jj >= i) ? vv[t] : 0.0f;
-                vv[t] = x;
-            }
-            *reinterpret_cast<float4*>(S + i * PLD + j) = make_float4(vv[0], vv[1], vv[2], vv[3]);
-        }
-    }
-    __syncthreads();
-    LLMC_STAMP(1);
-    for (int kb = 0; kb < 4; ++kb) {
-        if (wv == 0) wave_potrf32_inv(PBLK(S, kb, kb), VBLK(kb, kb), rowbuf, lane, k0 + kb * 32, info);
-        __syncthreads();
-        LLMC_STAMP(2 + 2 * kb);
-        {
-            const int jb = kb + 1 + wv;
-            if (jb < 4) {
-                f32x16 acc = blk_mm<true>(VBLK(kb, kb), PBLK(S, kb, jb), zero, lane);
-                blk_store(PBLK(S, kb, jb), acc, lane, 1.0f);
-            }
-        }
-        __syncthreads();
-        {
-            int idx = 0;
-            for (int ib = kb + 1; ib < 4; ++ib)
-                for (int jb = ib; jb < 4; ++jb, ++idx)
-                    if ((idx & 3) == wv) {
-                        f32x16 acc = blk_mm<true>(PBLK(S, kb, ib), PBLK(S, kb, jb), zero, lane);
-                        blk_sub(PBLK(S, ib, jb), acc, lane);
-                    }
-        }
-        __syncthreads();
-        LLMC_STAMP(3 + 2 * kb);
-    }
-    if (nb == NB && (ld % 4 == 0) && (k0 % 4 == 0)) {
-#pragma unroll
-        for (int q = 0; q < 16; ++q) {
-            const int e4 = tid + 256 * q;
-            const int i = e4 >> 5, j = (e4 & 31) * 4;
-            float4 s4 = make_float4(0.f, 0.f, 0.f, 0.f);
-            if ((j >> 5) >= (i >> 5)) s4 = *reinterpret_cast<const float4*>(S + i * PLD + j);
-            *reinterpret_cast<float4*>(W + (int64_t)(k0 + i) * ld + k0 + j) = s4;
-        }
-    } else {
-        for (int e = tid; e < NB * NB; e += 256) {
-            const int i = e >> 7, j = e & 127;
-            if (i < nb && j < nb) W[(int64_t)(k0 + i) * ld + k0 + j] = (j >= i) ? S[i * PLD + j] : 0.0f;
-        }
-    }
-    LLMC_STAMP(10);
-    if (wv < 2) {
-        const int a = 2 * wv, b = a + 1;
-        f32x16 x = blk_mm<false>(VBLK(a, a), PBLK(S, a, b), zero, lane);
-        blk_store(VBLK(a, b), x, lane, 1.0f);
-        f32x16 y = blk_mm<false>(VBLK(a, b), VBLK(b, b), zero, lane);
-        blk_store(VBLK(a, b), y, lane, -1.0f);
-    }
-    __syncthreads();
-    {
-        const int r = wv >> 1, c = 2 + (wv & 1);
-        f32x16 x = blk_mm<false>(VBLK(r, r), PBLK(S, r, c), zero, lane);
-        if (r == 0) x = blk_mm<false>(VBLK(0, 1), PBLK(S, 1, c), x, lane);
-        __syncthreads();
-        blk_store(VBLK(r, c), x, lane, 1.0f);
-    }
-    __syncthreads();
-    {
-        const int r = wv >> 1, c = 2 + (wv & 1);
-        f32x16 y = blk_mm<false>(VBLK(r, 2), VBLK(2, c), zero, lane);
-        if (c == 3) y = blk_mm<false>(VBLK(r, 3), VBLK(3, 3), y, lane);
-        blk_store(PBLK(S, r, c), y, lane, -1.0f);
-    }
-    __syncthreads();
-    LLMC_STAMP(11);
-#pragma unroll
-    for (int q = 0; q < 16; ++q) {
-        const int e4 = tid + 256 * q;
-        const int i = e4 >> 5, j = (e4 & 31) * 4;
-        const int bi = i >> 5, bj = j >> 5;
-        float4 v4 = make_float4(0.f, 0.f, 0.f, 0.f);
-        if (bi == bj) v4 = *reinterpret_cast<const float4*>(Vd + (i & 31) * PLD + j);
-        else if (bi < 2 && bj >= 2) v4 = *reinterpret_cast<const float4*>(S + i * PLD + j);
-        else if (bi < bj) v4 = *reinterpret_cast<const float4*>(S + (bj * 32 + (i & 31)) * PLD + bi * 32 + (j & 31));
-        *reinterpret_cast<float4*>(Vout + i * NB + j) = v4;
-    }
-    LLMC_STAMP(12);
+#include "potrf_inv_body.h"
+}
+
+struct G3wRiders {
+    G3wArgs w;
+    int n;
+    uint16_t tile[RIDERS_CAP];
+};
+__global__ __launch_bounds__(256, 2) void k_potrf_inv_riders(float* __restrict__ W, int64_t ld, int k0, int nb, float* __restrict__ Vout,
+                                                          int* __restrict__ info, const G3wRiders r) {
+    extern __shared__ __attribute__((aligned(16))) char smem_g[];
+    if (blockIdx.x == 0) {
+        float* plds = reinterpret_cast<float*>(smem_g);
+#include "potrf_inv_body.h"
+        return;
+    }
+    if ((int)blockIdx.x > r.n) return;
+    const G3wArgs& a = r.w;
+    const int t = r.tile[blockIdx.x - 1];
+    const int ti = t >> 8, tj = t & 255;
+#include "gemm3w_tile_body.h"
 }
 #undef PBLK
 
@@ -570,6 +469,7 @@
 struct FactorCall {
     float* Wk; float* Vbuf; float* Xbuf; void* G6buf; int K; size_t xbuf_bytes;
     bool x3, planes, merge_far, g6;
+    int riders;
     float* at(int64_t r, int64_t c) const { return Wk + r * K + c; }
     float* V(int c0) const { return Vbuf + (size_t)(c0 / NB) * NB * NB; }
     static SgemmArgs one(int M, int N, int Kd, int epilogue) {
@@ -600,6 +500,11 @@
     bool split_planes(int k0, int oend, int r0) const {
         const int nfar = K - oend;
         return x3 && planes && nfar % 8 == 0 && (size_t)3 * (oend - k0) * nfar * 2 <= xbuf_bytes && gemm3_route(far(k0, oend, r0, K, true), true).planes();
+    }
+    int rider_cut(int k0, int oend) const {
+        const int mt = opt(OPT_GEMM3S_MIN_TILES);
+        const int T = K % NB ? 0 : rider_rows(K, oend, riders, mt > 0 ? mt : (riders + 1) / 2);
+        return T > 0 && gemm3_route(far(k0, oend, K - T * NB, K, true), true).g3w_form ? K - T * NB : K;
     }
     Level level(int64_t h) const {
         Level l{h, 2 * h * ((int64_t)K + 1), h, (int)((K - h + 2 * h - 1) / (2 * h)), 0, false, false};
@@ -633,10 +538,12 @@
 
 enum { CP_TRANSPOSE = 0, CP_POTRF = 1, CP_SOLVE = 2, CP_UPDATE = 3, CP_SPLIT = 4, CP_FAR = 7, CP_PLACE = 8, CP_ZERO = 9, CP_INV_X = 10,
        CP_INV_C = 11, CP_W = 22 };
+enum { CP_TILES = 12, CRP_BLOCK = CP_W, CRP_N, CRP_CUT, CRP_W, CRP_PER_ROW = 20 };
 enum { F_KERNEL = 0, F_SGEMM = 1, F_GEMM3 = 2, F_GEMM6 = 3 };
 struct Rect { int32_t buf, r0, r1, c0, c1; };
-static const int32_t CP_BLANK[CP_W] = {0, 0, -1, 0, 0, 0, 0, -1, 0, 0, 0, 0, -1, 0, 0, 0, 0, -1, 0, 0, 0, 0};
+static const int32_t CP_BLANK[CRP_W] = {0, 0, -1, 0, 0, 0, 0, -1, 0, 0, 0, 0, -1, 0, 0, 0, 0, -1, 0, 0, 0, 0, -1, 0, 0};
 static constexpr int POTRF_LDS = (NB * PLD + 32 * PLD + 64) * (int)sizeof(float);
+static_assert(POTRF_LDS >= G_LDS, "k_potrf_inv_riders reserves the factor role's LDS: a rider's tile must fit in it");
 static int launched() { LLMC_LAUNCH_CHECK(); return LLMC_OK; }
 struct FactorSink {
     const FactorCall& o; const Lanes& ln; PlanRec* rec; const float* other; const char* ws_end; int32_t* info;
@@ -651,10 +558,21 @@
         const int64_t n = v ? NB : o.K, off = f - (v ? o.Vbuf : w ? o.Wk : other);
         return Rect{ld != n ? -2 : v ? 1 : w ? 0 : 4, (int32_t)(off / n), (int32_t)(off / n + rows), (int32_t)(off % n), (int32_t)(off % n + cols)};
     }
-    int add(int kind, int form, Lane lane, Rect w, Rect a = Rect{-1}, Rect b = Rect{-1}, Rect w2 = Rect{-1}) const {
-        int32_t v[CP_W] = {kind, form};
+    int add(int kind, int form, Lane lane, Rect w, Rect a = Rect{-1}, Rect b = Rect{-1}, Rect w2 = Rect{-1}, const G3wRiders* rd = nullptr) const {
+        int32_t v[CRP_W] = {kind, form};
         memcpy(v + 2, &w, sizeof w), memcpy(v + 7, &a, sizeof a), memcpy(v + 12, &b, sizeof b), memcpy(v + 17, &w2, sizeof w2);
+        v[CRP_BLOCK] = -1;
+        if (!rd) return rec->row(v, ln.lane_of(ln.s[lane])), LLMC_OK;
+        const int cut = rect(rd->w.C, o.K, 1, 1).r0;
+        v[CRP_BLOCK] = o.K - (int)(rd->w.row2 / 2) - rd->w.nst * G_K, v[CRP_N] = rd->n, v[CRP_CUT] = cut;
         rec->row(v, ln.lane_of(ln.s[lane]));
+        for (int i = 0; i < rd->n; i += CRP_PER_ROW) {
+            int32_t t[CRP_W];
+            memcpy(t, CP_BLANK, sizeof t);
+            t[0] = CP_TILES, t[1] = rd->n - i < CRP_PER_ROW ? rd->n - i : CRP_PER_ROW;
+            for (int e = 0; e < t[1]; ++e) t[2 + e] = (cut / NB + (rd->tile[i + e] >> 8)) << 16 | (cut / NB + (rd->tile[i + e] & 255));
+            rec->row(t, ln.lane_of(ln.s[lane]));
+        }
         return LLMC_OK;
     }
     int transpose(const float* in, float* out, int upper_only) const {
@@ -662,10 +580,11 @@
         hipLaunchKernelGGL(k_antitranspose, dim3((o.K + 31) / 32, (o.K + 31) / 32), dim3(256), 0, ln.s[CHAIN], in, out, o.K, upper_only);
         return launched();
     }
-    int potrf(int c0, int nb) const {
+    int potrf(int c0, int nb, const G3wRiders* rd) const {
         float* Vb = o.V(c0);
-        if (rec) return add(CP_POTRF, F_KERNEL, CHAIN, rect(o.at(c0, c0), o.K, nb, nb), rect(o.at(c0, c0), o.K, nb, nb), Rect{-1}, rect(Vb, NB, nb, NB));
-        hipLaunchKernelGGL(k_potrf_inv, dim3(1), dim3(256), POTRF_LDS, ln.s[CHAIN], o.Wk, (int64_t)o.K, c0, nb, Vb, info);
+        if (rec) return add(CP_POTRF, F_KERNEL, CHAIN, rect(o.at(c0, c0), o.K, nb, nb), rect(o.at(c0, c0), o.K, nb, nb), Rect{-1}, rect(Vb, NB, nb, NB), rd);
+        if (rd) hipLaunchKernelGGL(k_potrf_inv_riders, dim3(1 + rd->n), dim3(256), POTRF_LDS, ln.s[CHAIN], o.Wk, (int64_t)o.K, c0, nb, Vb, info, *rd);
+        else hipLaunchKernelGGL(k_potrf_inv, dim3(1), dim3(256), POTRF_LDS, ln.s[CHAIN], o.Wk, (int64_t)o.K, c0, nb, Vb, info);
         return launched();
     }
     int product(int kind, const SgemmArgs& g, int form, bool TA, Lane lane) const {
@@ -706,7 +625,7 @@
     }
 };
 
-static int chol_inv_upper_impl(float* A, float* Uout, int64_t K64, void* ws, int32_t* info_dev, llmc_stream_t stream, PlanRec* rec = nullptr) {
+static int chol_inv_upper_impl(float* A, float* Uout, int64_t K64, void* ws, int32_t* info_dev, llmc_stream_t stream, PlanRec* rec = nullptr, int ncu = 0) {
     LLMC_REQUIRE(A && ws && info_dev && K64 > 0, "chol_inv_upper: null/empty argument");
     LLMC_REQUIRE(K64 % 4 == 0 && K64 < (1 << 30), "chol_inv_upper: K must be a multiple of 4");
     LLMC_REQUIRE(((uintptr_t)A & 15) == 0 && ((uintptr_t)ws & 255) == 0, "chol_inv_upper: alignment");
@@ -714,23 +633,40 @@
     const bool rev = Uout != nullptr;
     const FactorWs l = factor_ws(K);
     char* const w = (char*)ws;
+    Lanes ln((hipStream_t)stream, rec);
+    int riders = 0;
+    if (!ln.piped() && !opt(OPT_K3_SPLIT_FAR) && opt(OPT_K3_NO_RIDERS) != 1 && (!rec || ncu > 0)) {
+        riders = (rec ? ncu : device_cu_count()) - 1;
+        if (opt(OPT_K3_NO_RIDERS) > 1 && opt(OPT_K3_NO_RIDERS) < riders) riders = opt(OPT_K3_NO_RIDERS);
+        if (riders > RIDERS_CAP) riders = RIDERS_CAP;
+    }
     const FactorCall o{rev ? A : (float*)(w + l.work), (float*)(w + l.vbuf), (float*)(w + l.xbuf), w + l.g6, K, l.xbuf_bytes,
-                       !opt(OPT_K3_FP32), !opt(OPT_K3_NO_PLANES), !opt(OPT_K3_SPLIT_FAR), !opt(OPT_K3_NO_GEMM6)};
-    Lanes ln((hipStream_t)stream, rec);
+                       !opt(OPT_K3_FP32), !opt(OPT_K3_NO_PLANES), !opt(OPT_K3_SPLIT_FAR), !opt(OPT_K3_NO_GEMM6), riders};
     const FactorSink sink{o, ln, rec, rev ? Uout : A, w + l.total, info_dev};
     LLMC_TRY(ln.fork());
     if (!rec) {
         LLMC_HIP_CHECK(hipMemsetAsync(info_dev, 0, 4, ln.s[CHAIN]));
         LLMC_TRY(ensure_dynamic_lds((const void*)k_potrf_inv, POTRF_LDS));
+        if (riders > 0) LLMC_TRY(ensure_dynamic_lds((const void*)k_potrf_inv_riders, POTRF_LDS));
     }
     if (!rev) LLMC_TRY(sink.transpose(A, o.Wk, 0));
     Piece pc[2];
     Ev planes_read{};
+    uint16_t queue[RIDER_QUEUE_MAX];
+    int qn = 0, qnext = 0;
+    G3wRiders rd{};
     for (int k0 = 0; k0 < K; k0 += NBO) {
         const int oend = k0 + NBO < K ? k0 + NBO : K;
         for (int c0 = k0; c0 < oend; c0 += NB) {
             const int nb = K - c0 < NB ? K - c0 : NB;
-            LLMC_TRY(sink.potrf(c0, nb));
+            const bool ride = qnext < qn;
+            if (ride) {
+                rd.n = rider_share(qn - qnext, (oend - c0) / NB);
+                LLMC_REQUIRE(rd.n <= o.riders && oend - k0 == NBO, "chol_inv_upper: rider queue out of step");
+                rider_deal(queue + qnext, rd.n, rd.tile);
+                qnext += rd.n;
+            }
+            LLMC_TRY(sink.potrf(c0, nb, ride ? &rd : nullptr));
             if (c0 + nb >= K) break;
             const int np = step_pieces(c0 + nb, oend, K, ln.piped(), pc);
             LLMC_TRY(sink.product(CP_SOLVE, o.panel_solve(c0, nb, pc[0].a0, pc[0].a1), F_SGEMM, true, CHAIN));
@@ -745,14 +681,19 @@
         LLMC_TRY(ln.order(BULK, CHAIN));
         const int np = far_pieces(oend, K, !ln.piped() && o.x3 && o.merge_far, pc);
         const bool planes = o.split_planes(k0, oend, pc[np - 1].a0);
+        const int cut = planes && np == 1 ? o.rider_cut(k0, oend) : K;
         if (planes) {
             LLMC_TRY(ln.wait(CHAIN, planes_read));
             LLMC_TRY(sink.split(k0, oend));
         }
         for (int i = 0; i < np; ++i) {
             if (pc[i].lane == BULK) LLMC_TRY(ln.order(CHAIN, BULK));
-            LLMC_TRY(sink.product(CP_FAR, o.far(k0, oend, pc[i].a0, pc[i].a1, planes), o.x3 ? F_GEMM3 : F_SGEMM, true, pc[i].lane));
+            LLMC_TRY(sink.product(CP_FAR, o.far(k0, oend, pc[i].a0, pc[i].a1 < cut ? pc[i].a1 : cut, planes), o.x3 ? F_GEMM3 : F_SGEMM, true, pc[i].lane));
             if (pc[i].lane == BULK) LLMC_TRY(ln.record(BULK, &planes_read));
+        }
+        if (cut < K) {
+            g3w_operands(o.far(k0, oend, cut, K, true), rd.w);
+            qn = rider_queue((K - cut) / NB, queue), qnext = 0;
         }
     }
     LLMC_TRY(sink.place_diag());
@@ -781,11 +722,17 @@
     return chol_inv_upper_impl(Arev, Uout, K64, ws, info_dev, stream);
 }
 
+static int chol_plan(int64_t K, int rev, PlanRec rec, int ncu) {
+    float* const base = (float*)(uintptr_t)((uint64_t)1 << 40);
+    const size_t span = (size_t)1 << 36;
+    const int rc = chol_inv_upper_impl(base, rev ? base + span : nullptr, K, base + 2 * span, (int32_t*)(base + 3 * span), nullptr, &rec, ncu);
+    return rc ? rc : rec.n;
+}
 extern "C" int llmc_test_chol_plan(int64_t K, int rev, int with_lanes, int32_t* out, int cap) {
     LLMC_REQUIRE(out && cap >= 0, "chol plan: null output");
-    PlanRec rec{out, cap, 0, CP_W, with_lanes != 0, CP_BLANK};
-    float* const base = (float*)(uintptr_t)((uint64_t)1 << 40);
-    const size_t span = (size_t)1 << 36;
-    const int rc = chol_inv_upper_impl(base, rev ? base + span : nullptr, K, base + 2 * span, (int32_t*)(base + 3 * span), nullptr, &rec);
-    return rc ? rc : rec.n;
-}
+    return chol_plan(K, rev, PlanRec{out, cap, 0, CP_W, with_lanes != 0, CP_BLANK}, 0);
+}
+extern "C" int llmc_test_chol_rider_plan(int64_t K, int rev, int ncu, int32_t* out, int cap) {
+    LLMC_REQUIRE(out && cap >= 0 && ncu >= 0, "chol rider plan: null output");
+    return chol_plan(K, rev, PlanRec{out, cap, 0, CRP_W, false, CP_BLANK}, ncu > 0 ? ncu : device_cu_count());
+}
diff --git a/llmc_amd/csrc/common.h b/llmc_amd/csrc/common.h
--- a/llmc_amd/csrc/common.h
+++ b/llmc_amd/csrc/common.h
@@ -66,6 +66,7 @@
     OPT_SGEMM_NO_WIDE,
     OPT_GEMM3_NO_WIDE,
     OPT_NO_RIDERS,
+    OPT_K3_NO_RIDERS,
     OPT_KV_SINK_MAX_GRID,
     OPT_BLOCK_INFLUENCE_MAX_GRID,
     OPT_COUNT
diff --git a/llmc_amd/csrc/gemm3_wide.hip b/llmc_amd/csrc/gemm3_wide.hip
--- a/llmc_amd/csrc/gemm3_wide.hip
+++ b/llmc_amd/csrc/gemm3_wide.hip
@@ -1,28 +1,7 @@
-#include "mfma_common.h"
-#include "sgemm.h"
+#include "gemm3w_tile.h"
 
 namespace llmc {
 namespace {
-
-constexpr int G_ROW = G_B * 2;
-constexpr int G_PLANE = G_K * G_ROW;
-constexpr int G_OPND = 3 * G_PLANE;
-constexpr int G_SLOT = 2 * G_OPND;
-constexpr int G_SLOTS = 3;
-static_assert(G_LDS == G_SLOTS * G_SLOT, "72 KiB");
-constexpr int G_PER_XCD = 64;
-
-struct G3wArgs {
-    const uint16_t* PA;
-    const uint16_t* PB;
-    float* C;
-    int64_t ldc;
-    uint32_t row2, ps2, rowC;
-    uint32_t bytesP, bytesC;
-    int nst;
-    int tm, tn, sbm, nsb, sm_log, sn_log;
-    int upper;
-};
 
 __global__ __launch_bounds__(256, 2) void k_gemm3w(const G3wArgs a) {
     extern __shared__ __attribute__((aligned(16))) char smem_g[];
@@ -34,149 +13,14 @@
     if (ti >= a.tm || tj >= a.tn) return;
     if (a.upper && tj < ti) return;
 
-    const int tid = threadIdx.x, lane = tid & 63;
-    const int wv = __builtin_amdgcn_readfirstlane(tid >> 6);
-    const int wm = wv >> 1, wn = wv & 1;
-#if defined(G3W_DBG) && G3W_DBG == 1
-    const auto dA = uniform_rsrc(a.PA, a.bytesP);
-    const auto dB = uniform_rsrc(a.PB, a.bytesP);
-#else
-    const auto dA = uniform_rsrc(a.PA + (int64_t)ti * G_B, a.bytesP);
-    const auto dB = uniform_rsrc(a.PB + (int64_t)tj * G_B, a.bytesP);
-#endif
-    const auto dC = uniform_rsrc(a.C + (int64_t)ti * G_B * a.ldc + (int64_t)tj * G_B, a.bytesC);
-    LDS_AS char* lds = (LDS_AS char*)smem_g;
-    const uint32_t lds0 = (uint32_t)(uintptr_t)lds;
-    const int nst = a.nst;
-
-    uint32_t vo;
-    {
-        const int r = lane >> 4, c = lane & 15;
-        const int cs = (((c >> 2) ^ r) << 2) | (c & 3);
-        vo = (uint32_t)r * a.row2 + (uint32_t)cs * 16u;
-    }
-    auto issue = [&](int j, uint32_t slot_off) {
-        const uint32_t k0 = (uint32_t)j * G_K;
-#pragma unroll
-        for (int t = 0; t < 6; ++t) {
-            const int op = t / 3, pl = t % 3;
-            const uint32_t so = (uint32_t)pl * a.ps2 + (k0 + 4u * (uint32_t)wv) * a.row2;
-            const uint32_t dst = lds0 + slot_off + (uint32_t)op * G_OPND + (uint32_t)pl * G_PLANE + (uint32_t)wv * 1024u;
-            if (op == 0) dma16_to(dA, vo, so, dst); else dma16_to(dB, vo, so, dst);
-        }
-    };
-
-    const int p = lane & 15;
-    const int trow = 8 * (lane >> 5) + (p >> 2);
-    const int sub = 32 * ((lane >> 4) & 1) + 8 * (p & 3);
-    int offA[2], offB[2];
-#pragma unroll
-    for (int b = 0; b < 2; ++b) {
-        offA[b] = trow * G_ROW + (((2 * wm + b) ^ (p >> 2)) << 6) + sub;
-        offB[b] = G_OPND + trow * G_ROW + (((2 * wn + b) ^ (p >> 2)) << 6) + sub;
-    }
-    s16x8 fa[2][2][3], fb[2][2][3];
-    auto rd = [&](auto setc, auto fc, LDS_AS char* base) {
-        constexpr int S = decltype(setc)::value, f = decltype(fc)::value;
-        constexpr int grp = f >> 2, e = f & 3, b = e & 1;
-        constexpr bool isA = grp == 0 ? e >= 2 : e < 2;
-        constexpr int pl = grp == 0 ? (isA ? 2 : 0) : grp == 1 ? (isA ? 0 : 2) : 1;
-        if constexpr (isA) fa[S][b][pl] = tr_frag<G_ROW>(base + offA[b], pl * G_PLANE);
-        else fb[S][b][pl] = tr_frag<G_ROW>(base + offB[b], pl * G_PLANE);
-    };
-
-    f32x16 acc[2][2];
-#pragma unroll
-    for (int m = 0; m < 2; ++m)
-#pragma unroll
-        for (int n = 0; n < 2; ++n)
-#pragma unroll
-            for (int r = 0; r < 16; ++r) acc[m][n][r] = 0.0f;
-
-    issue(0, 0);
-    issue(1, G_SLOT);
-    issue(2, 2 * G_SLOT);
-    vm_wait<12>();
-    __builtin_amdgcn_s_barrier();
-    static_for<0, 12>([&](auto fc) { rd(std::integral_constant<int, 0>{}, fc, lds); });
-    __builtin_amdgcn_sched_barrier(0);
-
-    const uint32_t voC = (uint32_t)(wm * 64 + 4 * (lane >> 5)) * a.rowC + (uint32_t)(wn * 64 + (lane & 31)) * 4u;
-    auto soC = [&](uint32_t rowC, int m, int n, int r) { return (uint32_t)(m * 32 + (r & 3) + 8 * (r >> 2)) * rowC + (uint32_t)n * 128u; };
-    f32x16 oldc[2][2];
-    uint32_t cur = 0;
-    auto stage = [&](auto setc, auto cbc, auto youngc, int j) {
-        constexpr int S = decltype(setc)::value, CB = decltype(cbc)::value, YOUNG = decltype(youngc)::value;
-        if (j + 2 < nst) vm_wait<YOUNG>(); else vm_wait<0>();
-        __builtin_amdgcn_s_barrier();
-#if !(defined(G3W_DBG) && G3W_DBG == 2)
-        if (j + 3 < nst) issue(j + 3, cur);
-#endif
-        const uint32_t nxt = cur + G_SLOT == G_LDS ? 0u : cur + G_SLOT;
-        LDS_AS char* nb = lds + nxt;
-        __builtin_amdgcn_sched_barrier(0);
-        static_for<0, 24>([&](auto ic) {
-            constexpr int i = decltype(ic)::value, q = i >> 2, m = (i >> 1) & 1, n = i & 1;
-            constexpr int TA = q == 0 ? 2 : q == 1 ? 0 : q == 2 ? 1 : q == 3 ? 1 : 0;
-            constexpr int TB = q == 0 ? 0 : q == 1 ? 2 : q == 2 ? 1 : q == 3 ? 0 : q == 4 ? 1 : 0;
-            acc[m][n] = Mfma<LLMC_BF16>::run(fa[S][m][TA], fb[S][n][TB], acc[m][n]);
-            if constexpr (i < 12) rd(std::integral_constant<int, S ^ 1>{}, std::integral_constant<int, i>{}, nb);
-#if !(defined(G3W_DBG) && G3W_DBG == 3)
-            if constexpr (CB >= 0 && i >= 12 && i < 20) {
-#pragma unroll
-                for (int e = 0; e < 2; ++e) {
-                    constexpr int r0 = 2 * (i - 12);
-                    oldc[CB >> 1][CB & 1][r0 + e] = __builtin_bit_cast(float, __builtin_amdgcn_raw_buffer_load_b32(dC, voC, soC(a.rowC, CB >> 1, CB & 1, r0 + e), 0));
-                }
-            }
-#endif
-            __builtin_amdgcn_sched_barrier(0);
-        });
-        cur = nxt;
-    };
-    constexpr std::integral_constant<int, 0> S0{};
-    constexpr std::integral_constant<int, 1> S1{};
-    constexpr std::integral_constant<int, -1> NOC{};
-    stage(S0, std::integral_constant<int, 0>{}, std::integral_constant<int, 6>{}, 0);
-    stage(S1, std::integral_constant<int, 1>{}, std::integral_constant<int, 22>{}, 1);
-    stage(S0, std::integral_constant<int, 2>{}, std::integral_constant<int, 38>{}, 2);
-    stage(S1, std::integral_constant<int, 3>{}, std::integral_constant<int, 38>{}, 3);
-    stage(S0, NOC, std::integral_constant<int, 38>{}, 4);
-    stage(S1, NOC, std::integral_constant<int, 22>{}, 5);
-    for (int j = 6; j < nst; j += 2) {
-        stage(S0, NOC, std::integral_constant<int, 6>{}, j);
-        stage(S1, NOC, std::integral_constant<int, 6>{}, j + 1);
-    }
-
-    uint32_t rowC2 = a.rowC;
-    asm volatile("" : "+s"(rowC2));
-#pragma unroll
-    for (int m = 0; m < 2; ++m)
-#pragma unroll
-        for (int n = 0; n < 2; ++n) {
-            if (a.upper && ti == tj && 2 * wn + n < 2 * wm + m) continue;
-#if defined(G3W_DBG) && G3W_DBG == 3
-            if (acc[m][n][0] != 12345.678f) continue;
-#endif
-#pragma unroll
-            for (int r = 0; r < 16; ++r) {
-                const float v = oldc[m][n][r] - acc[m][n][r];
-                __builtin_amdgcn_raw_buffer_store_b32(__builtin_bit_cast(unsigned, v), dC, voC, soC(rowC2, m, n, r), 0);
-            }
-        }
+#include "gemm3w_tile_body.h"
 }
 
 }
 
 int gemm3w_launch(const SgemmArgs& a, const GemmRoute& r, hipStream_t st) {
     G3wArgs w{};
-    w.PA = (const uint16_t*)a.planesA; w.PB = (const uint16_t*)a.planesB; w.C = a.C; w.ldc = a.ldc;
-    w.row2 = (uint32_t)(a.ldp * 2); w.ps2 = (uint32_t)(a.plane_stride * 2); w.rowC = (uint32_t)(a.ldc * 4);
-    w.bytesP = (uint32_t)((2 * a.plane_stride + (int64_t)(a.Kd - 1) * a.ldp + G_B) * 2);
-    w.bytesC = (uint32_t)(((int64_t)(G_B - 1) * a.ldc + G_B) * 4);
-    w.nst = a.Kd / G_K;
-    w.tm = a.M / G_B; w.tn = a.N / G_B;
-    w.upper = a.c_upper_only ? 1 : 0;
+    g3w_operands(a, w);
     w.sm_log = r.sm_log; w.sn_log = r.sn_log; w.sbm = r.sbm; w.nsb = r.nsb;
     if (int rc = ensure_dynamic_lds((const void*)k_gemm3w, G_LDS)) return rc;
     hipLaunchKernelGGL(k_gemm3w, dim3(r.gx), dim3(r.threads), G_LDS, st, w);
diff --git a/llmc_amd/csrc/gemm3w_tile.h b/llmc_amd/csrc/gemm3w_tile.h
--- /dev/null
+++ b/llmc_amd/csrc/gemm3w_tile.h
@@ -0,0 +1,38 @@
+#pragma once
+#include "mfma_common.h"
+#include "sgemm.h"
+
+namespace llmc {
+namespace {
+
+constexpr int G_ROW = G_B * 2;
+constexpr int G_PLANE = G_K * G_ROW;
+constexpr int G_OPND = 3 * G_PLANE;
+constexpr int G_SLOT = 2 * G_OPND;
+constexpr int G_SLOTS = 3;
+static_assert(G_LDS == G_SLOTS * G_SLOT, "72 KiB");
+constexpr int G_PER_XCD = 64;
+
+struct G3wArgs {
+    const uint16_t* PA;
+    const uint16_t* PB;
+    float* C;
+    int64_t ldc;
+    uint32_t row2, ps2, rowC;
+    uint32_t bytesP, bytesC;
+    int nst;
+    int tm, tn, sbm, nsb, sm_log, sn_log;
+    int upper;
+};
+
+static inline void g3w_operands(const SgemmArgs& a, G3wArgs& w) {
+    w.PA = (const uint16_t*)a.planesA; w.PB = (const uint16_t*)a.planesB; w.C = a.C; w.ldc = a.ldc;
+    w.row2 = (uint32_t)(a.ldp * 2); w.ps2 = (uint32_t)(a.plane_stride * 2); w.rowC = (uint32_t)(a.ldc * 4);
+    w.bytesP = (uint32_t)((2 * a.plane_stride + (int64_t)(a.Kd - 1) * a.ldp + G_B) * 2);
+    w.bytesC = (uint32_t)(((int64_t)(G_B - 1) * a.ldc + G_B) * 4);
+    w.nst = a.Kd / G_K;
+    w.tm = a.M / G_B; w.tn = a.N / G_B;
+    w.upper = a.c_upper_only ? 1 : 0;
+}
+}
+}
diff --git a/llmc_amd/csrc/gemm3w_tile_body.h b/llmc_amd/csrc/gemm3w_tile_body.h
--- /dev/null
+++ b/llmc_amd/csrc/gemm3w_tile_body.h
@@ -0,0 +1,130 @@
+    const int tid = threadIdx.x, lane = tid & 63;
+    const int wv = __builtin_amdgcn_readfirstlane(tid >> 6);
+    const int wm = wv >> 1, wn = wv & 1;
+#if defined(G3W_DBG) && G3W_DBG == 1
+    const auto dA = uniform_rsrc(a.PA, a.bytesP);
+    const auto dB = uniform_rsrc(a.PB, a.bytesP);
+#else
+    const auto dA = uniform_rsrc(a.PA + (int64_t)ti * G_B, a.bytesP);
+    const auto dB = uniform_rsrc(a.PB + (int64_t)tj * G_B, a.bytesP);
+#endif
+    const auto dC = uniform_rsrc(a.C + (int64_t)ti * G_B * a.ldc + (int64_t)tj * G_B, a.bytesC);
+    LDS_AS char* lds = (LDS_AS char*)smem_g;
+    const uint32_t lds0 = (uint32_t)(uintptr_t)lds;
+    const int nst = a.nst;
+
+    uint32_t vo;
+    {
+        const int r = lane >> 4, c = lane & 15;
+        const int cs = (((c >> 2) ^ r) << 2) | (c & 3);
+        vo = (uint32_t)r * a.row2 + (uint32_t)cs * 16u;
+    }
+    auto issue = [&](int j, uint32_t slot_off) {
+        const uint32_t k0 = (uint32_t)j * G_K;
+#pragma unroll
+        for (int t = 0; t < 6; ++t) {
+            const int op = t / 3, pl = t % 3;
+            const uint32_t so = (uint32_t)pl * a.ps2 + (k0 + 4u * (uint32_t)wv) * a.row2;
+            const uint32_t dst = lds0 + slot_off + (uint32_t)op * G_OPND + (uint32_t)pl * G_PLANE + (uint32_t)wv * 1024u;
+            if (op == 0) dma16_to(dA, vo, so, dst); else dma16_to(dB, vo, so, dst);
+        }
+    };
+
+    const int p = lane & 15;
+    const int trow = 8 * (lane >> 5) + (p >> 2);
+    const int sub = 32 * ((lane >> 4) & 1) + 8 * (p & 3);
+    int offA[2], offB[2];
+#pragma unroll
+    for (int b = 0; b < 2; ++b) {
+        offA[b] = trow * G_ROW + (((2 * wm + b) ^ (p >> 2)) << 6) + sub;
+        offB[b] = G_OPND + trow * G_ROW + (((2 * wn + b) ^ (p >> 2)) << 6) + sub;
+    }
+    s16x8 fa[2][2][3], fb[2][2][3];
+    auto rd = [&](auto setc, auto fc, LDS_AS char* base) {
+        constexpr int S = decltype(setc)::value, f = decltype(fc)::value;
+        constexpr int grp = f >> 2, e = f & 3, b = e & 1;
+        constexpr bool isA = grp == 0 ? e >= 2 : e < 2;
+        constexpr int pl = grp == 0 ? (isA ? 2 : 0) : grp == 1 ? (isA ? 0 : 2) : 1;
+        if constexpr (isA) fa[S][b][pl] = tr_frag<G_ROW>(base + offA[b], pl * G_PLANE);
+        else fb[S][b][pl] = tr_frag<G_ROW>(base + offB[b], pl * G_PLANE);
+    };
+
+    f32x16 acc[2][2];
+#pragma unroll
+    for (int m = 0; m < 2; ++m)
+#pragma unroll
+        for (int n = 0; n < 2; ++n)
+#pragma unroll
+            for (int r = 0; r < 16; ++r) acc[m][n][r] = 0.0f;
+
+    issue(0, 0);
+    issue(1, G_SLOT);
+    issue(2, 2 * G_SLOT);
+    vm_wait<12>();
+    __builtin_amdgcn_s_barrier();
+    static_for<0, 12>([&](auto fc) { rd(std::integral_constant<int, 0>{}, fc, lds); });
+    __builtin_amdgcn_sched_barrier(0);
+
+    const uint32_t voC = (uint32_t)(wm * 64 + 4 * (lane >> 5)) * a.rowC + (uint32_t)(wn * 64 + (lane & 31)) * 4u;
+    auto soC = [&](uint32_t rowC, int m, int n, int r) { return (uint32_t)(m * 32 + (r & 3) + 8 * (r >> 2)) * rowC + (uint32_t)n * 128u; };
+    f32x16 oldc[2][2];
+    uint32_t cur = 0;
+    auto stage = [&](auto setc, auto cbc, auto youngc, int j) {
+        constexpr int S = decltype(setc)::value, CB = decltype(cbc)::value, YOUNG = decltype(youngc)::value;
+        if (j + 2 < nst) vm_wait<YOUNG>(); else vm_wait<0>();
+        __builtin_amdgcn_s_barrier();
+#if !(defined(G3W_DBG) && G3W_DBG == 2)
+        if (j + 3 < nst) issue(j + 3, cur);
+#endif
+        const uint32_t nxt = cur + G_SLOT == G_LDS ? 0u : cur + G_SLOT;
+        LDS_AS char* nb = lds + nxt;
+        __builtin_amdgcn_sched_barrier(0);
+        static_for<0, 24>([&](auto ic) {
+            constexpr int i = decltype(ic)::value, q = i >> 2, m = (i >> 1) & 1, n = i & 1;
+            constexpr int TA = q == 0 ? 2 : q == 1 ? 0 : q == 2 ? 1 : q == 3 ? 1 : 0;
+            constexpr int TB = q == 0 ? 0 : q == 1 ? 2 : q == 2 ? 1 : q == 3 ? 0 : q == 4 ? 1 : 0;
+            acc[m][n] = Mfma<LLMC_BF16>::run(fa[S][m][TA], fb[S][n][TB], acc[m][n]);
+            if constexpr (i < 12) rd(std::integral_constant<int, S ^ 1>{}, std::integral_constant<int, i>{}, nb);
+#if !(defined(G3W_DBG) && G3W_DBG == 3)
+            if constexpr (CB >= 0 && i >= 12 && i < 20) {
+#pragma unroll
+                for (int e = 0; e < 2; ++e) {
+                    constexpr int r0 = 2 * (i - 12);
+                    oldc[CB >> 1][CB & 1][r0 + e] = __builtin_bit_cast(float, __builtin_amdgcn_raw_buffer_load_b32(dC, voC, soC(a.rowC, CB >> 1, CB & 1, r0 + e), 0));
+                }
+            }
+#endif
+            __builtin_amdgcn_sched_barrier(0);
+        });
+        cur = nxt;
+    };
+    constexpr std::integral_constant<int, 0> S0{};
+    constexpr std::integral_constant<int, 1> S1{};
+    constexpr std::integral_constant<int, -1> NOC{};
+    stage(S0, std::integral_constant<int, 0>{}, std::integral_constant<int, 6>{}, 0);
+    stage(S1, std::integral_constant<int, 1>{}, std::integral_constant<int, 22>{}, 1);
+    stage(S0, std::integral_constant<int, 2>{}, std::integral_constant<int, 38>{}, 2);
+    stage(S1, std::integral_constant<int, 3>{}, std::integral_constant<int, 38>{}, 3);
+    stage(S0, NOC, std::integral_constant<int, 38>{}, 4);
+    stage(S1, NOC, std::integral_constant<int, 22>{}, 5);
+    for (int j = 6; j < nst; j += 2) {
+        stage(S0, NOC, std::integral_constant<int, 6>{}, j);
+        stage(S1, NOC, std::integral_constant<int, 6>{}, j + 1);
+    }
+
+    uint32_t rowC2 = a.rowC;
+    asm volatile("" : "+s"(rowC2));
+#pragma unroll
+    for (int m = 0; m < 2; ++m)
+#pragma unroll
+        for (int n = 0; n < 2; ++n) {
+            if (a.upper && ti == tj && 2 * wn + n < 2 * wm + m) continue;
+#if defined(G3W_DBG) && G3W_DBG == 3
+            if (acc[m][n][0] != 12345.678f) continue;
+#endif
+#pragma unroll
+            for (int r = 0; r < 16; ++r) {
+                const float v = oldc[m][n][r] - acc[m][n][r];
+                __builtin_amdgcn_raw_buffer_store_b32(__builtin_bit_cast(unsigned, v), dC, voC, soC(rowC2, m, n, r), 0);
+            }
+        }
diff --git a/llmc_amd/csrc/gemm_route.hip b/llmc_amd/csrc/gemm_route.hip
--- a/llmc_amd/csrc/gemm_route.hip
+++ b/llmc_amd/csrc/gemm_route.hip
@@ -41,7 +41,7 @@
     const int v = opt(OPT_SGEMM_NO_WIDE);
     return v == 1 ? 0 : v == 4 && a.M % 256 == 0 ? 4 : 2;
 }
-bool gemm3s_eligible(const SgemmArgs& a) {
+bool gemm3s_form(const SgemmArgs& a) {
     if (opt(OPT_GEMM3_NOSPEC)) return false;
     if (a.a_upper || a.a_lower || a.b_upper) return false;
     if ((((uintptr_t)a.C) & 15) || a.ldc % 4 || a.sC % 4) return false;
@@ -51,17 +51,24 @@
     if (a.Kd % (2 * G3K) || a.Kd_last % (2 * G3K) || a.Kd < 4 * G3K || a.Kd_last < 4 * G3K) return false;
     if (pre && (a.batch != 1 || a.ldp % 8 || a.plane_stride % 8 || (((uintptr_t)a.planesA | (uintptr_t)a.planesB) & 15))) return false;
     const int64_t extent = pre ? (2 * a.plane_stride + (kd + G3K) * a.ldp) * 2 : (kd + G3K) * (a.lda > a.ldb ? a.lda : a.ldb) * 4;
-    if (extent >= (int64_t)0x7fffff00) return false;
+    return extent < (int64_t)0x7fffff00;
+}
+bool gemm3s_eligible(const SgemmArgs& a) {
+    if (!gemm3s_form(a)) return false;
+    const bool pre = a.planesA != nullptr;
     const int64_t tm = (a.M + S_BM - 1) / S_BM, tn = (a.N + S_BN - 1) / S_BN;
     const int64_t tiles = a.c_upper_only ? tm * tn - tm * (tm - 1) : tm * tn;
     const int mt = opt(OPT_GEMM3S_MIN_TILES);
     const int min_tiles = mt > 0 ? mt : (pre ? 48 : 256);
     return tiles * a.batch >= min_tiles;
 }
-bool gemm3w_eligible(const SgemmArgs& a) {
+bool gemm3w_form(const SgemmArgs& a) {
     if (opt(OPT_GEMM3_NO_WIDE)) return false;
     if (!a.planesA || !a.planesB || a.epilogue != SG_SUB || a.M % G_B || a.N % G_B) return false;
-    if ((2 * a.plane_stride + ((int64_t)a.Kd + G_K) * a.ldp) * 2 >= (int64_t)0x7fffff00 || (int64_t)G_B * a.ldc * 4 >= (int64_t)0x7fffff00) return false;
+    return (2 * a.plane_stride + ((int64_t)a.Kd + G_K) * a.ldp) * 2 < (int64_t)0x7fffff00 && (int64_t)G_B * a.ldc * 4 < (int64_t)0x7fffff00;
+}
+bool gemm3w_eligible(const SgemmArgs& a) {
+    if (!gemm3w_form(a)) return false;
     const int64_t tm = a.M / G_B, tn = a.N / G_B;
     const int64_t tiles = a.c_upper_only ? tm * tn - tm * (tm - 1) / 2 : tm * tn;
     const int mt = opt(OPT_GEMM3S_MIN_TILES);
@@ -102,6 +109,7 @@
         ((uintptr_t)a.B & 15) || (a.sA % 4) || (a.sB % 4))
         return refuse(r, LLMC_EINVAL, "gemm3: operands must be 16-B aligned with ld and sizes multiples of 4");
     if ((const void*)a.C == (const void*)a.B || (const void*)a.C == (const void*)a.A) return refuse(r, LLMC_EINVAL, "gemm3: no in-place product");
+    r.g3w_form = TA && gemm3s_form(a) && gemm3w_form(a);
     if (!TA || !gemm3s_eligible(a)) return tiles(r, GK_GEMM3, a, G3B, G3B);
     if (gemm3w_eligible(a)) return tile_blocks(r, GK_GEMM3W, a.M / G_B, a.N / G_B, 6, a.c_upper_only != 0, G_LDS);
     r.threads = 512; r.lds = S_LDS; r.planes_dma = opt(OPT_GEMM3S_NO_DMA) ? 0 : 1;
diff --git a/llmc_amd/csrc/potrf_inv_body.h b/llmc_amd/csrc/potrf_inv_body.h
--- /dev/null
+++ b/llmc_amd/csrc/potrf_inv_body.h
@@ -0,0 +1,124 @@
+    float* S = plds;
+    float* Vd = plds + NB * PLD;
+    float* rowbuf = plds + NB * PLD + 32 * PLD;
+    const int tid = threadIdx.x;
+    const int lane = tid & 63;
+    const int wv = __builtin_amdgcn_readfirstlane(tid >> 6);
+    const f32x16 zero = {0.f, 0.f, 0.f, 0.f, 0.f, 0.f, 0.f, 0.f, 0.f, 0.f, 0.f, 0.f, 0.f, 0.f, 0.f, 0.f};
+    LLMC_STAMP(0);
+    {
+        float4 ld4[16];
+        const bool full = nb == NB && (ld % 4 == 0) && (k0 % 4 == 0);
+        if (full) {
+            const float* base = W + (int64_t)(k0 + (tid >> 5)) * ld + k0 + (tid & 31) * 4;
+#pragma unroll
+            for (int q = 0; q < 16; ++q) ld4[q] = *reinterpret_cast<const float4*>(base + (int64_t)(8 * q) * ld);
+        } else {
+#pragma unroll
+            for (int q = 0; q < 16; ++q) {
+                const int e4 = tid + 256 * q;
+                const int i = e4 >> 5, j = (e4 & 31) * 4;
+                float4 v = make_float4(0.f, 0.f, 0.f, 0.f);
+                if (i < nb) {
+                    const float* p = W + (int64_t)(k0 + i) * ld + k0 + j;
+                    if (j < nb) v.x = p[0];
+                    if (j + 1 < nb) v.y = p[1];
+                    if (j + 2 < nb) v.z = p[2];
+                    if (j + 3 < nb) v.w = p[3];
+                }
+                ld4[q] = v;
+            }
+        }
+#pragma unroll
+        for (int q = 0; q < 16; ++q) {
+            const int e4 = tid + 256 * q;
+            const int i = e4 >> 5, j = (e4 & 31) * 4;
+            float vv[4] = {ld4[q].x, ld4[q].y, ld4[q].z, ld4[q].w};
+#pragma unroll
+            for (int t = 0; t < 4; ++t) {
+                const int jj = j + t;
+                float x = (i == jj) ? 1.0f : 0.0f;
+                if (i < nb && jj < nb) x = (jj >= i) ? vv[t] : 0.0f;
+                vv[t] = x;
+            }
+            *reinterpret_cast<float4*>(S + i * PLD + j) = make_float4(vv[0], vv[1], vv[2], vv[3]);
+        }
+    }
+    __syncthreads();
+    LLMC_STAMP(1);
+    for (int kb = 0; kb < 4; ++kb) {
+        if (wv == 0) wave_potrf32_inv(PBLK(S, kb, kb), VBLK(kb, kb), rowbuf, lane, k0 + kb * 32, info);
+        __syncthreads();
+        LLMC_STAMP(2 + 2 * kb);
+        {
+            const int jb = kb + 1 + wv;
+            if (jb < 4) {
+                f32x16 acc = blk_mm<true>(VBLK(kb, kb), PBLK(S, kb, jb), zero, lane);
+                blk_store(PBLK(S, kb, jb), acc, lane, 1.0f);
+            }
+        }
+        __syncthreads();
+        {
+            int idx = 0;
+            for (int ib = kb + 1; ib < 4; ++ib)
+                for (int jb = ib; jb < 4; ++jb, ++idx)
+                    if ((idx & 3) == wv) {
+                        f32x16 acc = blk_mm<true>(PBLK(S, kb, ib), PBLK(S, kb, jb), zero, lane);
+                        blk_sub(PBLK(S, ib, jb), acc, lane);
+                    }
+        }
+        __syncthreads();
+        LLMC_STAMP(3 + 2 * kb);
+    }
+    if (nb == NB && (ld % 4 == 0) && (k0 % 4 == 0)) {
+#pragma unroll
+        for (int q = 0; q < 16; ++q) {
+            const int e4 = tid + 256 * q;
+            const int i = e4 >> 5, j = (e4 & 31) * 4;
+            float4 s4 = make_float4(0.f, 0.f, 0.f, 0.f);
+            if ((j >> 5) >= (i >> 5)) s4 = *reinterpret_cast<const float4*>(S + i * PLD + j);
+            *reinterpret_cast<float4*>(W + (int64_t)(k0 + i) * ld + k0 + j) = s4;
+        }
+    } else {
+        for (int e = tid; e < NB * NB; e += 256) {
+            const int i = e >> 7, j = e & 127;
+            if (i < nb && j < nb) W[(int64_t)(k0 + i) * ld + k0 + j] = (j >= i) ? S[i * PLD + j] : 0.0f;
+        }
+    }
+    LLMC_STAMP(10);
+    if (wv < 2) {
+        const int a = 2 * wv, b = a + 1;
+        f32x16 x = blk_mm<false>(VBLK(a, a), PBLK(S, a, b), zero, lane);
+        blk_store(VBLK(a, b), x, lane, 1.0f);
+        f32x16 y = blk_mm<false>(VBLK(a, b), VBLK(b, b), zero, lane);
+        blk_store(VBLK(a, b), y, lane, -1.0f);
+    }
+    __syncthreads();
+    {
+        const int r = wv >> 1, c = 2 + (wv & 1);
+        f32x16 x = blk_mm<false>(VBLK(r, r), PBLK(S, r, c), zero, lane);
+        if (r == 0) x = blk_mm<false>(VBLK(0, 1), PBLK(S, 1, c), x, lane);
+        __syncthreads();
+        blk_store(VBLK(r, c), x, lane, 1.0f);
+    }
+    __syncthreads();
+    {
+        const int r = wv >> 1, c = 2 + (wv & 1);
+        f32x16 y = blk_mm<false>(VBLK(r, 2), VBLK(2, c), zero, lane);
+        if (c == 3) y = blk_mm<false>(VBLK(r, 3), VBLK(3, 3), y, lane);
+        blk_store(PBLK(S, r, c), y, lane, -1.0f);
+    }
+    __syncthreads();
+    LLMC_STAMP(11);
+#pragma unroll
+    for (int q = 0; q < 16; ++q) {
+        const int e4 = tid + 256 * q;
+        const int i = e4 >> 5, j = (e4 & 31) * 4;
+        const int bi = i >> 5, bj = j >> 5;
+        float4 v4 = make_float4(0.f, 0.f, 0.f, 0.f);
+        if (bi == bj) v4 = *reinterpret_cast<const float4*>(Vd + (i & 31) * PLD + j);
+        else if (bi < 2 && bj >= 2) v4 = *reinterpret_cast<const float4*>(S + i * PLD + j);
+        else if (bi < bj) v4 = *reinterpret_cast<const float4*>(S + (bj * 32 + (i & 31)) * PLD + bi * 32 + (j & 31));
+        *reinterpret_cast<float4*>(Vout + i * NB + j) = v4;
+    }
+    LLMC_STAMP(12);
diff --git a/llmc_amd/csrc/sgemm.h b/llmc_amd/csrc/sgemm.h
--- a/llmc_amd/csrc/sgemm.h
+++ b/llmc_amd/csrc/sgemm.h
@@ -40,6 +40,7 @@
     int planes_dma;
     int sm_log, sn_log, sbm, nsb;
     int wide_form;
+    bool g3w_form;
     bool planes() const { return status == LLMC_OK && !empty && (kernel == GK_GEMM3S_PRE || kernel == GK_GEMM3W); }
 };
 GemmRoute sgemm_route(const SgemmArgs& a, bool TA, bool TB);
```

New measurement: 79.39, median of 6. Within noise of the previous version (+0.7%).
